# RVC-Project/obs-rvc

Hardware: AMD Instinct MI355X
Metric: audio frames/sec (10 ms hops of new input, 160 ms chunks @16 kHz) (higher is better)
Workload: dtype f32; 1 GPU; BASELINE configs[1]: 1 stream(s)/GPU, ContentVec v2-768 + RMVPE + NSF-HiFiGAN v2-48k, retrieval off, preset full; streams_per_gpu=1, streams_total=1, hip_graph=False

## Files before the change

include/rvc_mi355x_debug.h:

```cpp
#ifndef RVC_MI355X_DEBUG_H
#define RVC_MI355X_DEBUG_H
#include "rvc_mi355x.h"
#ifdef __cplusplus
extern "C" {
#endif

int rvc_debug_option(const char *name, const char *value);
int rvc_debug_stamps(rvc_engine *e, char *buf, size_t cap);
int rvc_debug_last_plan(rvc_engine *e, int *n_ops);
int rvc_debug_profile_dump(rvc_engine *e, char *buf, size_t cap);
double rvc_debug_conv_check(rvc_engine *e, int M, int Cin, int KW, int dil, int N, int streams, int pre_act);
double rvc_debug_conv2d_check(rvc_engine *e, int M, int Cin, int H, int W, int streams, int kind, int residual);
double rvc_debug_ln_fold_check(rvc_engine *e, int M, int K, int N, float offset);
typedef struct rvc_debug_layer_spec {
    int form, streams;
    int cin, cout, kw, stride, pad, dil, groups;
    int t_in, t_out, x_halo, y_halo, r_halo;
    int act; float slope; float scale; int accumulate;
    int pre_act; float pre_slope;
    int no_bias, final_out, glu;
    int res;
    int n, kws[4], dils[4], pads[4];
    int x_grouped, res_grouped, y_ws;
} rvc_debug_layer_spec;
int rvc_debug_layer(rvc_engine *e, const rvc_debug_layer_spec *s, const float *w, const float *bias, float *x, float *y, float *r, long long *geo);
typedef struct rvc_debug_op_spec {
    int op, streams;
    int E, heads, T, window, C, H;
    int x_halo, y_halo;
    int reps, graph;
} rvc_debug_op_spec;
int rvc_debug_op(rvc_engine *e, const rvc_debug_op_spec *s, const float *w0, const float *w1, float *x, float *y, int *status, long long *geo);
typedef struct rvc_debug_stream_state {
    float uppower; unsigned stream_id, chunk; int status;
    float cache_pitchf[1024];
} rvc_debug_stream_state;
typedef struct rvc_debug_front_spec {
    int op, streams, graph;
    int n, frame;
    float bn_scale, bn_shift;
    int C, L;
    int Tm, update, shift, cache_start, read_start, R;
    int T, upp, x_halo, f0_num, f0_den;
    float sr, lin_w, lin_b;
    unsigned seed;
} rvc_debug_front_spec;
int rvc_debug_front(rvc_engine *e, const rvc_debug_front_spec *s, const float *w0, const float *w1, float *const *buf, rvc_debug_stream_state *state, long long *geo);
int rvc_debug_autotune_dump(char *buf, size_t cap);
void rvc_debug_autotune_reset(void);
int rvc_debug_weight_slabs(int device, int *count, size_t *bytes);
const char *rvc_debug_last_kernel(void);
int rvc_debug_formant_table(size_t o, size_t n, float *out, size_t cap, size_t *width);
float rvc_debug_session_sola_ms(rvc_session *s, int enable);

#ifdef __cplusplus
}
#endif
#endif
```

obs_rvc_amd/csrc/engine.hip:

```cpp
#include "engine_int.h"
#include "../../include/rvc_mi355x_debug.h"
#include "crossfade.hip.h"
#include <chrono>

static bool g_planted_queues = false;
__attribute__((constructor)) static void rvc_runtime_defaults()
{
    if (getenv("RVC_NO_RUNTIME_DEFAULTS")) return;
    if (!getenv("GPU_MAX_HW_QUEUES")) { setenv("GPU_MAX_HW_QUEUES", "16", 0); g_planted_queues = true; }
}

namespace rvc {

static void init_kernel_attrs()
{
    static std::mutex mu; static bool done[64] = {};
    int dev = 0; HIPCHK(hipGetDevice(&dev));
    std::lock_guard<std::mutex> lk(mu);
    if (dev >= 0 && dev < 64) { if (done[dev]) return; done[dev] = true; }
    plan_kernel_attrs(); retrieval_kernel_attrs();
}

static void init_constants(rvc_engine *e)
{
// ... 1107 lines not shown
        HIPCHK(hipEventRecord(b, e->stream));
        HIPCHK(hipStreamSynchronize(e->stream));
        float ms; HIPCHK(hipEventElapsedTime(&ms, a, b));
        us = ms * 1e3 / iters;
        (void)hipEventDestroy(a); (void)hipEventDestroy(b);
        free_conv(cw);
        return RVC_OK;
    });
    return us;
}
#endif

double rvc_debug_ln_fold_check(rvc_engine *e, int M, int K, int N, float offset)
{
    double worst = -1.0;
    (void)guarded(e, [&]() {
        if (K % 16 != 0) throw ShapeError("K must be a multiple of 16");
        auto rnd = [](size_t i, unsigned salt) { return (float)((((i + 1) * 2654435761u) ^ (salt * 40503u) ^ (i >> 5)) % 2001) / 1000.0f - 1.0f; };
        std::vector<float> w1((size_t)M * K), b1(M), w2((size_t)K * M), b2(K), g(K), beta(K), hx((size_t)K * N), hz((size_t)M * N);
        for (size_t i = 0; i < w1.size(); i++) w1[i] = 0.5f * rnd(i, 1);
        for (size_t i = 0; i < w2.size(); i++) w2[i] = 0.5f * rnd(i, 2);
        for (int m = 0; m < M; m++) b1[m] = 0.1f * rnd(m, 3);
        for (int k = 0; k < K; k++) { b2[k] = 0.1f * rnd(k, 4); g[k] = 1.0f + 0.3f * rnd(k, 5); beta[k] = 0.2f * rnd(k, 6); }
        for (size_t i = 0; i < hx.size(); i++) hx[i] = 2.0f * rnd(i, 7) + offset;
        for (size_t i = 0; i < hz.size(); i++) hz[i] = rnd(i, 8);
        float *wsum = nullptr;
        ConvW c1 = ModelCV::fold_ln(w1.data(), b1.data(), M, K, g.data(), beta.data(), &wsum);
        ConvW c2 = prep_conv(w2.data(), b2.data(), K, M, 1, 1);
        float *dg = upload_f(g), *dbeta = upload_f(beta);
        Plan pl; pl.B = 1;
        T1 x = make_t1(pl.arena, 1, K, N, 0), y1 = make_t1(pl.arena, 1, M, N, 0), z = make_t1(pl.arena, 1, M, N, 0), y2 = make_t1(pl.arena, 1, K, N, 0);
        float *st = pl.arena.floats((size_t)2 * N + 16);
        for (int k = 0; k < K; k++) HIPCHK(hipMemcpy(x.p + (long long)k * x.ld, &hx[(size_t)k * N], (size_t)N * 4, hipMemcpyHostToDevice));
        for (int m = 0; m < M; m++) HIPCHK(hipMemcpy(z.p + (long long)m * z.ld, &hz[(size_t)m * N], (size_t)N * 4, hipMemcpyHostToDevice));
        { ConvOpts o; o.ln_wsum = wsum; o.ln_stats_out = st; o.ln_rows = K; add_conv1d(pl, c1, x, y1, 1, 0, 1, o); }
        { ConvOpts o; o.res = x.p; o.res_cs = x.ld; o.res_bs = x.bs; o.ln_stats_in = st; o.ln_g = dg; o.ln_b = dbeta; add_conv1d(pl, c2, z, y2, 1, 0, 1, o); }
        HIPCHK(hipDeviceSynchronize());
        for (auto &op : pl.ops.v) op(e->stream);
        HIPCHK(hipStreamSynchronize(e->stream));
        HIPCHK(hipGetLastError());
        std::vector<double> ln((size_t)K * N), mean(N), rstd(N);
        for (int n = 0; n < N; n++) {
            double s = 0; for (int k = 0; k < K; k++) s += hx[(size_t)k * N + n];
            const double mu = s / K; double q = 0;
            for (int k = 0; k < K; k++) { const double d = hx[(size_t)k * N + n] - mu; q += d * d; }
            mean[n] = mu; rstd[n] = 1.0 / std::sqrt(q / K + 1e-5);
            for (int k = 0; k < K; k++) ln[(size_t)k * N + n] = (hx[(size_t)k * N + n] - mu) * rstd[n] * g[k] + beta[k];
        }
        double err = 0.0;
        std::vector<float> row(N), hst((size_t)2 * N);
        {
            double ss = 0; std::vector<double> ref((size_t)M * N);
            for (int m = 0; m < M; m++) for (int n = 0; n < N; n++) {
                double a = b1[m]; for (int k = 0; k < K; k++) a += (double)w1[(size_t)m * K + k] * ln[(size_t)k * N + n];
                ref[(size_t)m * N + n] = a; ss += a * a;
            }
            const double rms1 = std::sqrt(ss / ((double)M * N)) + 1e-12;
            for (int m = 0; m < M; m++) {
                HIPCHK(hipMemcpy(row.data(), y1.p + (long long)m * y1.ld, (size_t)N * 4, hipMemcpyDeviceToHost));
                for (int n = 0; n < N; n++) err = std::max(err, std::fabs((double)row[n] - ref[(size_t)m * N + n]) / rms1);
            }
        }
        {
            double ss = 0; std::vector<double> ref((size_t)K * N);
            for (int k = 0; k < K; k++) for (int n = 0; n < N; n++) {
                double a = b2[k]; for (int m = 0; m < M; m++) a += (double)w2[(size_t)k * M + m] * hz[(size_t)m * N + n];
                a += ln[(size_t)k * N + n];
                ref[(size_t)k * N + n] = a; ss += a * a;
            }
            const double rms2 = std::sqrt(ss / ((double)K * N)) + 1e-12;
            for (int k = 0; k < K; k++) {
                HIPCHK(hipMemcpy(row.data(), y2.p + (long long)k * y2.ld, (size_t)N * 4, hipMemcpyDeviceToHost));
                for (int n = 0; n < N; n++) err = std::max(err, std::fabs((double)row[n] - ref[(size_t)k * N + n]) / rms2);
            }
        }
        HIPCHK(hipMemcpy(hst.data(), st, (size_t)2 * N * 4, hipMemcpyDeviceToHost));
        for (int n = 0; n < N; n++) {
            err = std::max(err, std::fabs((double)hst[2 * n] - mean[n]) / (std::fabs(mean[n]) + 1.0));
            err = std::max(err, std::fabs((double)hst[2 * n + 1] - rstd[n]) / rstd[n]);
        }
        worst = err;
        free_conv(c1); free_conv(c2);
        wfree(wsum); wfree(dg); wfree(dbeta);
        return RVC_OK;
    });
    return worst;
}

#ifdef RVC_TUNING
int rvc_debug_conv_probe(rvc_engine *e, int M, int Cin, int KW, int dil, int N, unsigned long long *out, size_t cap_waves, double *event_us, int *waves_per_wg)
{
    int nw = -1;
    (void)guarded(e, [&]() {
        std::vector<float> w((size_t)M * Cin * KW), bias(M, 0.1f);
        for (size_t i = 0; i < w.size(); i++) w[i] = (float)((i * 2654435761u) % 1000) / 1000.0f - 0.5f;
        ConvW cw = prep_conv(w.data(), bias.data(), M, Cin, KW, 1);
        Plan pl; pl.B = 1;
        const int pad = (KW - 1) * dil / 2;
        T1 x = make_t1(pl.arena, 1, Cin, N, (pad + 3) / 4 * 4), y = make_t1(pl.arena, 1, M, N, 0);
        std::vector<float> hx((size_t)Cin * x.ld, 0.25f);
        HIPCHK(hipMemcpy(x.p - x.halo, hx.data(), hx.size() * 4, hipMemcpyHostToDevice));
        unsigned long long *d_probe; const size_t pbytes = (size_t)1 << 24;
        HIPCHK(hipMalloc(&d_probe, pbytes)); HIPCHK(hipMemset(d_probe, 0, pbytes));
        g_kprobe = d_probe;
        ConvOpts o; if (const char *a = tune_env("RVC_BENCH_ACT")) o.act = atoi(a);
        add_conv1d(pl, cw, x, y, 1, pad, dil, o);
        g_kprobe = nullptr;
        HIPCHK(hipDeviceSynchronize());
        for (int i = 0; i < 5; i++) for (auto &op : pl.ops.v) op(e->stream);
        HIPCHK(hipDeviceSynchronize());
        HIPCHK(hipMemset(d_probe, 0, pbytes));
        HIPCHK(hipDeviceSynchronize());
        pl.profile = true; pl.prof_used = 0;
        for (auto &op : pl.ops.v) op(e->stream);
        HIPCHK(hipDeviceSynchronize());
        float t = 0.f; HIPCHK(hipEventElapsedTime(&t, pl.prof[0].a, pl.prof[0].b));
        if (event_us) *event_us = t * 1e3;
        nw = g_last_wgs * g_last_waves;
        if (waves_per_wg) *waves_per_wg = g_last_waves;
        if ((size_t)nw <= cap_waves && (size_t)nw * 128 <= pbytes) HIPCHK(hipMemcpy(out, d_probe, (size_t)nw * 128, hipMemcpyDeviceToHost));
        else nw = -2;
        (void)hipFree(d_probe);
        free_conv(cw);
        return RVC_OK;
    });
    return nw;
}
#endif

double rvc_debug_conv_check(rvc_engine *e, int M, int Cin, int KW, int dil, int N, int streams, int pre_act)
{
    double worst = -1.0;
    (void)guarded(e, [&]() {
        std::vector<float> w((size_t)M * Cin * KW), bias(M);
        for (size_t i = 0; i < w.size(); i++) w[i] = (float)((i * 2654435761u) % 1000) / 1000.0f - 0.5f;
        for (int m = 0; m < M; m++) bias[m] = 0.01f * (float)(m % 7) - 0.02f;
        ConvW cw = prep_conv(w.data(), bias.data(), M, Cin, KW, 1);
        Plan pl; pl.B = streams;
        const int pad = (KW - 1) * dil / 2, halo = (pad + 3) / 4 * 4;
        T1 x = make_t1(pl.arena, streams, Cin, N, halo), y = make_t1(pl.arena, streams, M, N, 0);
        std::vector<float> hx((size_t)streams * Cin * N);
        for (size_t i = 0; i < hx.size(); i++) hx[i] = (float)(((i * 40503u) ^ (i >> 3)) % 2001) / 1000.0f - 1.0f;
        for (int b = 0; b < streams; b++)
            for (int c = 0; c < Cin; c++)
                HIPCHK(hipMemcpy(x.p + (long long)b * x.bs + (long long)c * x.ld, &hx[((size_t)b * Cin + c) * N], (size_t)N * 4, hipMemcpyHostToDevice));
        ConvOpts o; if (pre_act) { o.pre_act = ACT_LRELU; o.pre_slope = 0.1f; }
        add_conv1d(pl, cw, x, y, 1, pad, dil, o);
        HIPCHK(hipDeviceSynchronize());
        for (auto &op : pl.ops.v) op(e->stream);
        HIPCHK(hipStreamSynchronize(e->stream));
        HIPCHK(hipGetLastError());
        std::vector<float> hy((size_t)streams * M * N);
        for (int b = 0; b < streams; b++)
            HIPCHK(hipMemcpy2D(&hy[(size_t)b * M * N], (size_t)N * 4, y.p + (long long)b * y.bs, (size_t)y.ld * 4, (size_t)N * 4, M, hipMemcpyDeviceToHost));
        const int nthr = (int)std::max(1u, std::min(16u, std::thread::hardware_concurrency()));
        std::vector<double> errs(nthr, 0.0), sss(nthr, 0.0);
        std::vector<std::thread> pool;
        for (int t = 0; t < nthr; t++)
            pool.emplace_back([&, t]() {
                std::vector<double> ref((size_t)N);
                for (long long bm = t; bm < (long long)streams * M; bm += nthr) {
                    const int b = (int)(bm / M), m = (int)(bm % M);
                    for (int n = 0; n < N; n++) {
                        double a = bias[m];
                        for (int c = 0; c < Cin; c++)
                            for (int k = 0; k < KW; k++) {
// ... 445 lines not shown
```

obs_rvc_amd/csrc/engine_int.h:

```cpp
#pragma once
#include "../../include/rvc_mi355x.h"
#include "blob.h"
#include "kernels.hip.h"
#include "formant.hip.h"
#include "igemm_launch.h"
#include <hip/hip_ext.h>

#include <algorithm>
#include <atomic>
#include <cmath>
#include <cstdarg>
#include <cstddef>
#include <functional>
#include <map>
#include <memory>
#include <mutex>
#include <string>
#include <tuple>
#include <vector>
#include <thread>

namespace rvc {

const char *test_opt(const char *name);
// ... 59 lines not shown
    size_t left_ = 0, total_ = 0;
};

struct T1 {
    float *p = nullptr;
    int B = 1, C = 0, T = 0, ld = 0, halo = 0;
    long long bs = 0;
    T1 rows(int c0, int n) const { T1 r = *this; r.p = p + (long long)c0 * ld; r.C = n; return r; }
};
struct T2 {
    float *p = nullptr;
    int B = 1, C = 0, H = 0, W = 0, ld = 0, cs = 0;
    long long bs = 0;
    T2 chans(int c0, int n) const { T2 r = *this; r.p = p + (long long)c0 * cs; r.C = n; return r; }
};

static inline size_t t1_guard(int ld) { return (size_t)ld + 64; }
static inline size_t t2_guard(int ld) { return (size_t)ld * 2 + 64; }
static inline T1 make_t1(Arena &a, int B, int C, int T, int halo)
{
    T1 t;
    t.B = B; t.C = C; t.T = T; t.halo = halo;
    t.ld = (T + 2 * halo + 3) / 4 * 4;
    t.bs = (long long)C * t.ld;
    const size_t guard = t1_guard(t.ld);
    float *base = a.floats((size_t)B * t.bs + 2 * guard);
    t.p = base + guard + halo;
    return t;
}
static inline T2 make_t2(Arena &a, int B, int C, int H, int W)
{
    T2 t;
    t.B = B; t.C = C; t.H = H; t.W = W;
    t.ld = W + 2;
    t.cs = (H + 2) * t.ld;
    t.bs = (long long)C * t.cs;
    const size_t guard = t2_guard(t.ld);
    float *base = a.floats((size_t)B * t.bs + 2 * guard);
    t.p = base + guard + t.ld + 1;
    return t;
}

struct ConvW {
    float *w = nullptr, *bias = nullptr;
    int M = 0, K = 0, Kp = 0, nphase = 1;
    int Cin = 0, Cout = 0, KW = 1, groups = 1;
    int S = 1, ntaps = 1;
    bool transposed = false;
    bool owns = true;
    std::vector<float> host_w;
};

static inline int round16(int k) { return (k + 15) / 16 * 16; }


void *wmalloc(size_t bytes); void wfree(void *p);
void *wmalloc_plan(size_t bytes);
void wslab_info(int dev, int *count, size_t *bytes);
float *upload_f(const std::vector<float> &v, int cls = 0);
float *upload_f(const float *p, size_t n);
float *upload_fragments(const std::vector<float> &panel, int nphase, int M, int Kp, int cls = 0);
static inline long long phase_stride(const ConvW &c) { return (long long)((c.M + 15) / 16 * 16) * c.Kp; }
ConvW prep_conv(const float *w, const float *bias, int Cout, int Cin, int KW, int groups);
ConvW prep_convT1d(const float *w, const float *bias, int Cin, int Cout, int K, int S);
ConvW prep_convT2d(const float *w, const float *bias, int Cin, int Cout);
void free_conv(ConvW &c);
const float *c32s_panel(const float *src_frag, int M, int nchunks, int cin, int KW);
void merge_convs(const std::vector<ConvW *> &cs);

constexpr int LN_FOLD_MAX_STREAMS = 1;

struct ConvOpts {
    int act = ACT_NONE; float slope = 0.f; float scale = 1.f; bool accumulate = false;
    int pre_act = ACT_NONE; float pre_slope = 0.f;
    const float *res = nullptr; int res_cs = 0; long long res_bs = 0; int res_rs = 0;
    int m_off = 0, m_cnt = -1;
    bool no_bias = false;
    bool glu = false;
    bool bf3 = false;
    int y_ws = 0;
    bool final_out = false;
    const float *ln_wsum = nullptr; float *ln_stats_out = nullptr; int ln_rows = 0;
    const float *ln_stats_in = nullptr, *ln_g = nullptr, *ln_b = nullptr;
};

struct ProfEvent { hipEvent_t a, b; double flops; double bytes; int desc = -1; };

struct Plan;
typedef std::function<void(hipStream_t)> Op;

struct TapRec { std::string name; int rank; T1 t1; T2 t2; };

struct OpList {
    std::vector<Op> v;
    std::vector<int> sid;
    std::vector<int> kind;
    std::vector<int> order_eager, order_graph;
    int cur = 0;
    void push_back(Op o) { v.push_back(std::move(o)); sid.push_back(cur); kind.push_back(0); }
    void fork(int s) { v.push_back(Op()); sid.push_back(s); kind.push_back(1); }
    void join(int s) { v.push_back(Op()); sid.push_back(s); kind.push_back(2); }
};

struct Plan {
    Arena arena;
    OpList ops;
    std::vector<TapRec> taps;
    int B = 1; size_t L = 0, frame16k = 0; uint32_t skip_head = 0, R = 0;
    int T = 0, Tm = 0, C = 0; size_t N = 0;
    bool with_index = false, with_taps = false;
    bool bucket = false;
    std::map<std::vector<int>, const int *> koff_tabs;
    bool rm_fuse = false;
    bool bf3 = false;
    bool autotune = false;
    double tune_ms = 0; int tuned_layers = 0, tune_changed = 0, tune_hits = 0;
    bool plain_plan = false;
    int mode = 0;
    uint32_t R2 = 0; bool fstage = false;
    int dec_frames() const { return fstage ? (int)R2 : (int)R; }
    float *d_in = nullptr;
    T1 cv_out, audio;
    float *d_f0 = nullptr;
    float *d_feat = nullptr;
    int *d_knn_idx = nullptr; float *d_knn_dist = nullptr;
    unsigned *knn_ticket = nullptr; size_t knn_ticket_bytes = 0;
    std::vector<Op> knn_fallback;
    size_t op_phone = 0, op_ret_begin = 0, op_ret_end = 0;
    unsigned opt_gen = 0;
    bool profile = false;
    std::vector<ProfEvent> prof;
    std::vector<std::string> descs;
    size_t prof_used = 0;
    double igemm_flops = 0;
    int n_igemm = 0;
    std::vector<float *> owned_dev;
    unsigned long long *d_stamps = nullptr; std::vector<std::string> stamp_names;
    int slot = 0; hipEvent_t ev_done = nullptr; bool ev_done_valid = false;
    const float *cur_in = nullptr; float *cur_out = nullptr; long long cur_out_bs = 0;
    bool in_direct_ok = true, out_direct_ok = false;
    bool final_out_honoured = false;
    hipGraphExec_t graph_exec = nullptr;
    ProfEvent *prof_slot(double flops, double bytes, int desc)
    {
        if (!profile) return nullptr;
        if (prof_used == prof.size()) { ProfEvent e; HIPCHK(hipEventCreate(&e.a)); HIPCHK(hipEventCreate(&e.b)); prof.push_back(e); }
        ProfEvent *pe = &prof[prof_used++];
        pe->flops = flops; pe->bytes = bytes; pe->desc = desc;
        return pe;
    }
    ~Plan()
    {
        for (float *p : owned_dev) wfree(p);
        if (graph_exec) (void)hipGraphExecDestroy(graph_exec);
        if (ev_done) (void)hipEventDestroy(ev_done);
        for (auto &e : prof) { (void)hipEventDestroy(e.a); (void)hipEventDestroy(e.b); }
    }
};


extern unsigned long long *g_kprobe;
extern int g_last_waves, g_last_wgs, g_ncu;
extern thread_local char g_last_kernel[32];
void queue_igemm(Plan &pl, IgemmP p, int B, const std::vector<int> &koff, const std::vector<PhaseD> &phases, bool final_out = false);
template <class Launch> void queue_gemm_launch(Plan &pl, const char *desc, double flops, int wgs, int waves, bool final_out, const IgemmP &p, Launch launch);
void fill_epilogue(IgemmP &p, const ConvW &cw, const ConvOpts &o);
void add_conv1d(Plan &pl, const ConvW &cw, const T1 &x, const T1 &y, int stride, int pad, int dil, ConvOpts o = ConvOpts());
void add_conv1d_multi(Plan &pl, const std::vector<const ConvW *> &cws, const T1 &x, bool x_grouped, const T1 &y,
                      const std::vector<int> &pads, const std::vector<int> &dils, ConvOpts o = ConvOpts(), bool res_grouped = true);
void add_conv1d_two(Plan &pl, const ConvW &c0, const ConvW &c1, const float *pair_bias, const T1 &x, const T1 &y0, const T1 &y1);
void add_convT1d(Plan &pl, const ConvW &cw, const T1 &x, const T1 &y, int pad, ConvOpts o = ConvOpts());
void add_conv2d(Plan &pl, const ConvW &cw, const T2 &x, const T2 &y, ConvOpts o = ConvOpts());
void add_convT2d(Plan &pl, const ConvW &cw, const T2 &x, const T2 &y, ConvOpts o = ConvOpts());
void add_layernorm(Plan &pl, const T1 &x, const float *g, const float *b);
void add_attention(Plan &pl, const T1 &qkv, const T1 &out, int heads);
void add_relpos_attention(Plan &pl, const T1 &qkv, const T1 &out, int heads, const float *rel_k, const float *rel_v, int window);
void add_gru(Plan &pl, const T1 &gi, const T1 &out, int H, const float *whh, const float *whhT, const float *bhh, int *status, int status_stride);
void add_stamp(Plan &pl, const char *name);
void add_tap(Plan &pl, const char *name, const T1 &t);
void add_tap2(Plan &pl, const char *name, const T2 &t);
void plan_kernel_attrs();
void retrieval_kernel_attrs();

struct DevVec { float *p = nullptr; };
static inline float *dv(const Blob &b, const std::string &name) { const BlobTensor &t = b.t(name); return upload_f(t.data, t.nelem); }

struct ModelCV {
    int conv_dim, embed, heads, ffn, run_layers, pos_k, pos_groups, out_dim;
    int conv_k[7], conv_s[7];
    ConvW conv[7], proj, pos, final_proj;
    float *gn_g, *gn_b, *ln0_g, *ln0_b, *encln_g, *encln_b;
    float *conv0_raw = nullptr;
    struct Layer { ConvW qkv, o, ff1, ff2, qkv_f, ff1_f; float *qkv_wsum = nullptr, *ff1_wsum = nullptr; float *ln1_g, *ln1_b, *ln2_g, *ln2_b; };
    bool has_folded = false;
    ConvW proj_f; float *proj_wsum = nullptr;
    static ConvW fold_ln(const float *w, const float *bias, int M, int K, const float *g, const float *beta, float **wsum_dev)
    {
        std::vector<float> wf((size_t)M * K), bf(M), ws(M);
        for (int m = 0; m < M; m++) {
            double sb = bias ? bias[m] : 0.0, sw = 0.0;
            for (int k = 0; k < K; k++) {
                const float v = w[(size_t)m * K + k] * g[k];
                wf[(size_t)m * K + k] = v;
                sb += (double)w[(size_t)m * K + k] * beta[k];
                sw += v;
            }
            bf[m] = (float)sb; ws[m] = (float)sw;
        }
        *wsum_dev = upload_f(ws);
        return prep_conv(wf.data(), bf.data(), M, K, 1, 1);
    }
    std::vector<Layer> layers;
    std::vector<float *> owned;
    size_t weight_bytes = 0;
    explicit ModelCV(const Blob &b)
    {
        conv_dim = b.icfg("conv_dim"); embed = b.icfg("embed"); heads = b.icfg("heads"); ffn = b.icfg("ffn");
        run_layers = b.icfg("run_layers"); pos_k = b.icfg("pos_k"); pos_groups = b.icfg("pos_groups"); out_dim = b.icfg("out_dim");
        int cin = 1;
        for (int i = 0; i < 7; i++) {
            conv_k[i] = b.icfg(fmt("conv_k%d", i)); conv_s[i] = b.icfg(fmt("conv_s%d", i));
            conv[i] = prep_conv(b.w(fmt("cv.conv%d.w", i)), nullptr, conv_dim, cin, conv_k[i], 1);
            cin = conv_dim;
        }
        auto own = [&](const std::string &n) { float *p = dv(b, n); owned.push_back(p); return p; };
        conv0_raw = own("cv.conv0.w");
        gn_g = own("cv.gn.g"); gn_b = own("cv.gn.b"); ln0_g = own("cv.ln0.g"); ln0_b = own("cv.ln0.b");
        proj = prep_conv(b.w("cv.proj.w"), b.w("cv.proj.b"), embed, conv_dim, 1, 1);
        pos = prep_conv(b.w("cv.pos.w"), b.w("cv.pos.b"), embed, embed, pos_k, pos_groups);
        encln_g = own("cv.enc_ln.g"); encln_b = own("cv.enc_ln.b");
        const int E = embed;
        for (int l = 0; l < run_layers; l++) {
            Layer L;
            std::vector<float> w((size_t)3 * E * E), bb((size_t)3 * E);
            const char *nm[3] = {"q", "k", "v"};
            for (int j = 0; j < 3; j++) {
                memcpy(&w[(size_t)j * E * E], b.w(fmt("cv.l%d.", l) + nm[j] + ".w"), (size_t)E * E * 4);
                memcpy(&bb[(size_t)j * E], b.w(fmt("cv.l%d.", l) + nm[j] + ".b"), (size_t)E * 4);
            }
            L.qkv = prep_conv(w.data(), bb.data(), 3 * E, E, 1, 1);
            L.o = prep_conv(b.w(fmt("cv.l%d.o.w", l)), b.w(fmt("cv.l%d.o.b", l)), E, E, 1, 1);
            L.ff1 = prep_conv(b.w(fmt("cv.l%d.ff1.w", l)), b.w(fmt("cv.l%d.ff1.b", l)), ffn, E, 1, 1);
            L.ff2 = prep_conv(b.w(fmt("cv.l%d.ff2.w", l)), b.w(fmt("cv.l%d.ff2.b", l)), E, ffn, 1, 1);
            L.ln1_g = own(fmt("cv.l%d.ln1.g", l)); L.ln1_b = own(fmt("cv.l%d.ln1.b", l));
            L.ln2_g = own(fmt("cv.l%d.ln2.g", l)); L.ln2_b = own(fmt("cv.l%d.ln2.b", l));
            if (E >= 256 && E % 64 == 0 && ffn % 64 == 0 && !test_opt("RVC_NO_LN_FUSE")) {
                has_folded = true;
                L.ff1_f = fold_ln(b.w(fmt("cv.l%d.ff1.w", l)), b.w(fmt("cv.l%d.ff1.b", l)), ffn, E, b.w(fmt("cv.l%d.ln1.g", l)), b.w(fmt("cv.l%d.ln1.b", l)), &L.ff1_wsum);
                if (l > 0) L.qkv_f = fold_ln(w.data(), bb.data(), 3 * E, E, b.w(fmt("cv.l%d.ln2.g", l - 1)), b.w(fmt("cv.l%d.ln2.b", l - 1)), &L.qkv_wsum);
                else L.qkv_f = fold_ln(w.data(), bb.data(), 3 * E, E, b.w("cv.enc_ln.g"), b.w("cv.enc_ln.b"), &L.qkv_wsum);
            }
            layers.push_back(L);
        }
        if (out_dim != E) final_proj = prep_conv(b.w("cv.final_proj.w"), b.w("cv.final_proj.b"), out_dim, E, 1, 1);
        if (has_folded && conv_dim % 64 == 0) proj_f = fold_ln(b.w("cv.proj.w"), b.w("cv.proj.b"), embed, conv_dim, b.w("cv.ln0.g"), b.w("cv.ln0.b"), &proj_wsum);
        weight_bytes = b.bytes();
    }
// ... 73 lines not shown
            r.f_w1 = upload_f(all); r.f_w2 = r.f_w1 + o2; r.f_sc = r.has_sc ? r.f_w1 + o3 : nullptr; r.f_lines = (int)(all.size() / 32);
        }
        return r;
    }
    explicit ModelRM(const Blob &b)
    {
        en_out = b.icfg("en_out"); levels = b.icfg("levels"); n_blocks = b.icfg("n_blocks"); inter_layers = b.icfg("inter_layers");
        n_mels = b.icfg("n_mels"); gru_hidden = b.icfg("gru_hidden"); n_out = b.icfg("n_out");
        bn_scale = b.w("rm.bn0")[0]; bn_shift = b.w("rm.bn0")[1];
        int ci = 1, co = en_out;
        for (int lv = 0; lv < levels; lv++) {
            std::vector<ResBlockW> v;
            for (int j = 0; j < n_blocks; j++) v.push_back(block(b, fmt("rm.enc%d.b%d.", lv, j), j == 0 ? ci : co, co));
            enc.push_back(v);
            ci = co; co *= 2;
        }
        for (int lv = 0; lv < inter_layers; lv++) {
            std::vector<ResBlockW> v;
            for (int j = 0; j < n_blocks; j++) v.push_back(block(b, fmt("rm.int%d.b%d.", lv, j), j == 0 ? (lv == 0 ? ci : co) : co, co));
            inter.push_back(v);
        }
        ci = co;
        for (int lv = 0; lv < levels; lv++) {
            co = ci / 2;
            up.push_back(prep_convT2d(b.w(fmt("rm.dec%d.up.w", lv)), b.w(fmt("rm.dec%d.up.b", lv)), ci, co));
            std::vector<ResBlockW> v;
            for (int j = 0; j < n_blocks; j++) v.push_back(block(b, fmt("rm.dec%d.b%d.", lv, j), j == 0 ? 2 * co : co, co));
            dec.push_back(v);
            ci = co;
        }
        cnn = prep_conv(b.w("rm.cnn.w"), b.w("rm.cnn.b"), 3, en_out, 9, 1);
        const int H = gru_hidden, I = 3 * n_mels;
        std::vector<float> wih((size_t)6 * H * I), bih((size_t)6 * H), bh((size_t)6 * H);
        const char *sfx[2] = {"f", "b"};
        const float *whh_dir[2];
        for (int d = 0; d < 2; d++) {
            memcpy(&wih[(size_t)d * 3 * H * I], b.w(std::string("rm.gru.w_ih_") + sfx[d]), (size_t)3 * H * I * 4);
            memcpy(&bih[(size_t)d * 3 * H], b.w(std::string("rm.gru.b_ih_") + sfx[d]), (size_t)3 * H * 4);
            memcpy(&bh[(size_t)d * 3 * H], b.w(std::string("rm.gru.b_hh_") + sfx[d]), (size_t)3 * H * 4);
            whh_dir[d] = b.w(std::string("rm.gru.w_hh_") + sfx[d]);
        }
        gru_ih = prep_conv(wih.data(), bih.data(), 6 * H, I, 1, 1);
        {
            std::vector<float> wt, wr;
            gru_prep_whh(whh_dir, H, wt, wr);
            whhT = upload_f(wt); bhh = upload_f(bh); whh = upload_f(wr);
        }
        fc = prep_conv(b.w("rm.fc.w"), b.w("rm.fc.b"), n_out, 2 * H, 1, 1);
        weight_bytes = b.bytes();
    }
    ~ModelRM()
    {
        auto fb = [](std::vector<std::vector<ResBlockW>> &vv) { for (auto &v : vv) for (auto &r : v) { free_conv(r.c1); free_conv(r.c2); free_conv(r.sc); if (r.pair_bias) wfree(r.pair_bias); if (r.f_w1) wfree(r.f_w1); } };
        fb(enc); fb(inter); fb(dec);
        for (auto &u : up) free_conv(u);
        free_conv(cnn); free_conv(gru_ih); free_conv(fc);
        if (whhT) wfree(whhT);
        if (bhh) wfree(bhh);
        if (whh) wfree(whh);
    }
};

template <typename T> static inline void glu_pack_rows(const T *w, const float *bias, int H, size_t K, std::vector<float> &wp, std::vector<float> &bp)
{
    if (H % 8 != 0) throw std::runtime_error("GLU-gated layer: channel count must be a multiple of 8");
    wp.resize((size_t)2 * H * K); bp.resize((size_t)2 * H);
    for (int r = 0; r < 2 * H; r++) {
        const int f = r >> 4, kq = (r & 15) >> 2, rr = r & 3;
        const int src = f * 8 + kq * 2 + (rr & 1) + (rr >= 2 ? H : 0);
        for (size_t q = 0; q < K; q++) wp[(size_t)r * K + q] = (float)w[(size_t)src * K + q];
        bp[r] = bias[src];
    }
}

struct ModelSY {
    int phone_dim, hidden, inter, filter, heads, enc_layers, enc_k, window, flow_n, wn_layers, wn_k, gin, up_init, n_ups, n_rb, n_rbd, sr;
    int up_rate[8], up_kernel[8], rb_k[8], rb_d[8];
    ConvW phone, proj;
    float *pitch_emb = nullptr;
    struct Layer {
        ConvW qkv, o, ff1, ff2, qkv_f; float *qkv_wsum = nullptr; float *rel_k, *rel_v, *ln1_g, *ln1_b, *ln2_g, *ln2_b;
    };
    ConvW proj_f; float *proj_wsum = nullptr; bool has_folded = false;
    std::vector<Layer> layers;
    struct Flow {
        ConvW pre, post; std::vector<ConvW> in, rs; bool flipped = false;
        std::vector<float> h_pre_w, h_pre_b, h_post_w, h_post_b;
        std::vector<std::vector<float>> h_in_w, h_in_b, h_rs_w, h_rs_b;
        ConvW pre1, postc, posth; std::vector<ConvW> inc; float *pair_bias = nullptr;
    };
    bool composed = false;
    std::vector<Flow> flows;
    ConvW dec_pre, dec_post;
    std::vector<ConvW> ups, ncs;
    std::vector<std::vector<std::vector<std::pair<ConvW, ConvW>>>> rbs;
    float src_w, src_b;
    std::vector<float *> owned;
    size_t weight_bytes = 0;
    explicit ModelSY(const Blob &b)
    {
        phone_dim = b.icfg("phone_dim"); hidden = b.icfg("hidden"); inter = b.icfg("inter"); filter = b.icfg("filter"); heads = b.icfg("heads");
        enc_layers = b.icfg("enc_layers"); enc_k = b.icfg("enc_k"); window = b.icfg("window"); flow_n = b.icfg("flow_n");
        wn_layers = b.icfg("wn_layers"); wn_k = b.icfg("wn_k"); gin = b.icfg("gin"); up_init = b.icfg("up_init"); n_ups = b.icfg("n_ups");
        n_rb = b.icfg("n_rb"); n_rbd = b.icfg("n_rbd"); sr = b.icfg("sr");
        for (int i = 0; i < n_ups; i++) { up_rate[i] = b.icfg(fmt("up_rate%d", i)); up_kernel[i] = b.icfg(fmt("up_kernel%d", i)); }
        for (int j = 0; j < n_rb; j++) rb_k[j] = b.icfg(fmt("rb_k%d", j));
        for (int m = 0; m < n_rbd; m++) rb_d[m] = b.icfg(fmt("rb_d%d", m));
        auto own = [&](const std::string &n) { float *p = dv(b, n); owned.push_back(p); return p; };
        const int H = hidden, G = gin;
        const float *g = b.w("sy.g");
        phone = prep_conv(b.w("sy.enc.phone.w"), b.w("sy.enc.phone.b"), H, phone_dim, 1, 1);
        pitch_emb = own("sy.enc.pitch_emb");
        for (int l = 0; l < enc_layers; l++) {
            Layer L;
            std::vector<float> w((size_t)3 * H * H), bb((size_t)3 * H);
            const char *nm[3] = {"q", "k", "v"};
            for (int j = 0; j < 3; j++) {
                memcpy(&w[(size_t)j * H * H], b.w(fmt("sy.enc.l%d.", l) + nm[j] + ".w"), (size_t)H * H * 4);
                memcpy(&bb[(size_t)j * H], b.w(fmt("sy.enc.l%d.", l) + nm[j] + ".b"), (size_t)H * 4);
            }
            L.qkv = prep_conv(w.data(), bb.data(), 3 * H, H, 1, 1);
            L.o = prep_conv(b.w(fmt("sy.enc.l%d.o.w", l)), b.w(fmt("sy.enc.l%d.o.b", l)), H, H, 1, 1);
            L.ff1 = prep_conv(b.w(fmt("sy.enc.l%d.ff1.w", l)), b.w(fmt("sy.enc.l%d.ff1.b", l)), filter, H, enc_k, 1);
            L.ff2 = prep_conv(b.w(fmt("sy.enc.l%d.ff2.w", l)), b.w(fmt("sy.enc.l%d.ff2.b", l)), H, filter, enc_k, 1);
            L.rel_k = own(fmt("sy.enc.l%d.rel_k", l)); L.rel_v = own(fmt("sy.enc.l%d.rel_v", l));
            L.ln1_g = own(fmt("sy.enc.l%d.ln1.g", l)); L.ln1_b = own(fmt("sy.enc.l%d.ln1.b", l));
            L.ln2_g = own(fmt("sy.enc.l%d.ln2.g", l)); L.ln2_b = own(fmt("sy.enc.l%d.ln2.b", l));
            if (H >= 128 && H % 16 == 0 && !test_opt("RVC_NO_LN_FUSE")) {
                has_folded = true;
                if (l > 0) L.qkv_f = ModelCV::fold_ln(w.data(), bb.data(), 3 * H, H, b.w(fmt("sy.enc.l%d.ln2.g", l - 1)), b.w(fmt("sy.enc.l%d.ln2.b", l - 1)), &L.qkv_wsum);
            }
            layers.push_back(L);
        }
        proj = prep_conv(b.w("sy.enc.proj.w"), b.w("sy.enc.proj.b"), 2 * inter, H, 1, 1);
        if (has_folded)
            proj_f = ModelCV::fold_ln(b.w("sy.enc.proj.w"), b.w("sy.enc.proj.b"), 2 * inter, H, b.w(fmt("sy.enc.l%d.ln2.g", enc_layers - 1)), b.w(fmt("sy.enc.l%d.ln2.b", enc_layers - 1)), &proj_wsum);
        const int half = inter / 2;
        for (int i = 0; i < flow_n; i++) {
            Flow F;
            F.flipped = ((flow_n - i) & 1) != 0;
            {
                std::vector<float> w((size_t)2 * H * half, 0.f), bb((size_t)2 * H, 0.f);
                const float *pw = b.w(fmt("sy.flow%d.pre.w", i)), *pb = b.w(fmt("sy.flow%d.pre.b", i));
                for (int r = 0; r < H; r++) {
                    bb[r] = pb[r];
                    for (int q = 0; q < half; q++) w[(size_t)r * half + q] = pw[(size_t)r * half + (F.flipped ? half - 1 - q : q)];
                }
                F.pre = prep_conv(w.data(), bb.data(), 2 * H, half, 1, 1);
                F.h_pre_w.assign(w.begin(), w.begin() + (size_t)H * half); F.h_pre_b.assign(bb.begin(), bb.begin() + H);
            }
            const float *cw = b.w(fmt("sy.flow%d.cond.w", i)), *cb = b.w(fmt("sy.flow%d.cond.b", i));
            for (int j = 0; j < wn_layers; j++) {
                std::vector<float> bias(2 * H);
                const float *ib = b.w(fmt("sy.flow%d.in%d.b", i, j));
                for (int r = 0; r < 2 * H; r++) {
                    float a = cb[j * 2 * H + r];
                    for (int q = 0; q < G; q++) a += cw[(size_t)(j * 2 * H + r) * G + q] * g[q];
                    bias[r] = ib[r] + a;
                }
                {
                    const float *iw = b.w(fmt("sy.flow%d.in%d.w", i, j));
                    const size_t Kin = (size_t)H * wn_k;
                    std::vector<float> w, pb;
                    glu_pack_rows(iw, bias.data(), H, Kin, w, pb);
                    F.in.push_back(prep_conv(w.data(), pb.data(), 2 * H, H, wn_k, 1));
                    F.h_in_w.emplace_back(iw, iw + (size_t)2 * H * Kin); F.h_in_b.push_back(bias);
                }
                int rs_c = j < wn_layers - 1 ? 2 * H : H;
                F.rs.push_back(prep_conv(b.w(fmt("sy.flow%d.rs%d.w", i, j)), b.w(fmt("sy.flow%d.rs%d.b", i, j)), rs_c, H, 1, 1));
                { const float *rw = b.w(fmt("sy.flow%d.rs%d.w", i, j)), *rb = b.w(fmt("sy.flow%d.rs%d.b", i, j)); F.h_rs_w.emplace_back(rw, rw + (size_t)rs_c * H); F.h_rs_b.emplace_back(rb, rb + rs_c); }
            }
            {
                const float *pw = b.w(fmt("sy.flow%d.post.w", i)), *pb = b.w(fmt("sy.flow%d.post.b", i));
                std::vector<float> w((size_t)half * H), bb(half);
                for (int r = 0; r < half; r++) {
                    const int src = F.flipped ? half - 1 - r : r;
                    memcpy(&w[(size_t)r * H], pw + (size_t)src * H, (size_t)H * sizeof(float));
                    bb[r] = pb[src];
                }
                F.post = prep_conv(w.data(), bb.data(), half, H, 1, 1);
                F.h_post_w = w; F.h_post_b = bb;
            }
            flows.push_back(F);
        }
        if (hidden % 16 == 0 && inter == hidden && !test_opt("RVC_NO_WN_COMPOSE")) compose_flows();
        {
            std::vector<float> bias(up_init);
            const float *cw = b.w("sy.dec.cond.w"), *cb = b.w("sy.dec.cond.b"), *pb = b.w("sy.dec.pre.b");
            for (int c = 0; c < up_init; c++) { float a = cb[c]; for (int q = 0; q < G; q++) a += cw[(size_t)c * G + q] * g[q]; bias[c] = pb[c] + a; }
            dec_pre = prep_conv(b.w("sy.dec.pre.w"), bias.data(), up_init, inter, 7, 1);
        }
        int c = up_init;
        for (int i = 0; i < n_ups; i++) {
            int co = c / 2;
            ups.push_back(prep_convT1d(b.w(fmt("sy.dec.up%d.w", i)), b.w(fmt("sy.dec.up%d.b", i)), c, co, up_kernel[i], up_rate[i]));
            int sf = 1; for (int q = i + 1; q < n_ups; q++) sf *= up_rate[q];
            int nk = i + 1 < n_ups ? 2 * sf : 1;
            ncs.push_back(prep_conv(b.w(fmt("sy.dec.nc%d.w", i)), b.w(fmt("sy.dec.nc%d.b", i)), co, 1, nk, 1));
            std::vector<std::vector<std::pair<ConvW, ConvW>>> stage;
            for (int j = 0; j < n_rb; j++) {
                std::vector<std::pair<ConvW, ConvW>> chain;
                for (int m = 0; m < n_rbd; m++) {
                    ConvW c1 = prep_conv(b.w(fmt("sy.dec.rb%d_%d.c1_%d.w", i, j, m)), b.w(fmt("sy.dec.rb%d_%d.c1_%d.b", i, j, m)), co, co, rb_k[j], 1);
                    ConvW c2 = prep_conv(b.w(fmt("sy.dec.rb%d_%d.c2_%d.w", i, j, m)), b.w(fmt("sy.dec.rb%d_%d.c2_%d.b", i, j, m)), co, co, rb_k[j], 1);
                    chain.push_back({c1, c2});
                }
                stage.push_back(chain);
            }
            rbs.push_back(stage);
            for (int m = 0; m < n_rbd && n_rb > 1; m++) {
                std::vector<ConvW *> a, bb;
                for (int j = 0; j < n_rb; j++) { a.push_back(&rbs.back()[j][m].first); bb.push_back(&rbs.back()[j][m].second); }
                merge_convs(a); merge_convs(bb);
            }
            c = co;
        }
        dec_post = prep_conv(b.w("sy.dec.post.w"), nullptr, 1, c, 7, 1);
        src_w = b.w("sy.src")[0]; src_b = b.w("sy.src")[1];
        weight_bytes = b.bytes();
// ... 35 lines not shown
                        }
                }
                std::vector<float> wp, pb;
                glu_pack_rows(w.data(), F.h_in_b[j].data(), H, (size_t)Cin * K5, wp, pb);
                WJ[fi][j] = std::move(wp); BJ[fi][j] = std::move(pb);
            }
        };
        auto one_flow = [&](int fi) {
            Flow &F = flows[fi];
            WP1[fi].assign((size_t)H * I, 0.f); BP1[fi] = F.h_pre_b;
            for (int r = 0; r < H; r++) for (int q = 0; q < half; q++) WP1[fi][(size_t)r * I + x0_row0(F) + q] = F.h_pre_w[(size_t)r * half + q];
            const int KA = nl * H, Kin = KA + I;
            std::vector<double> pc((size_t)half * KA, 0.0), pcb(half, 0.0);
            for (int r = 0; r < half; r++) {
                double bacc = F.h_post_b[r];
                for (int j = 0; j < nl; j++) {
                    const int row0 = j < nl - 1 ? H : 0;
                    const float *S = F.h_rs_w[j].data() + (size_t)row0 * H, *sb = F.h_rs_b[j].data() + row0;
                    for (int h = 0; h < H; h++) {
                        const double v = F.h_post_w[(size_t)r * H + h];
                        for (int c = 0; c < H; c++) pc[(size_t)r * KA + (size_t)j * H + c] += v * S[(size_t)h * H + c];
                        bacc += v * sb[h];
                    }
                }
                pcb[r] = bacc;
            }
            const bool has_next = fi > 0;
            const int r1 = x1_row0(F);
            std::vector<double> wz((size_t)I * Kin, 0.0), bz(I, 0.0);
            for (int c = 0; c < I; c++) wz[(size_t)c * Kin + KA + c] = 1.0;
            for (int r = 0; r < half; r++) {
                for (int q = 0; q < KA; q++) wz[(size_t)(r1 + r) * Kin + q] = -pc[(size_t)r * KA + q];
                bz[r1 + r] = -pcb[r];
            }
            WM[fi].resize(wz.size()); BM[fi].resize(I);
            for (size_t q = 0; q < wz.size(); q++) WM[fi][q] = (float)wz[q];
            for (int r = 0; r < I; r++) BM[fi][r] = (float)bz[r];
            if (has_next) {
                const Flow &N = flows[fi - 1];
                std::vector<double> wh((size_t)H * Kin, 0.0);
                WH[fi].resize(wh.size()); BH[fi].resize(H);
                for (int r = 0; r < H; r++) {
                    double bacc = N.h_pre_b[r];
                    for (int q = 0; q < half; q++) {
                        const double v = N.h_pre_w[(size_t)r * half + q];
                        const int zc = x0_row0(N) + q;
                        wh[(size_t)r * Kin + KA + zc] += v;
                        if (zc >= r1 && zc < r1 + half) {
                            const int pr = zc - r1;
                            for (int c = 0; c < KA; c++) wh[(size_t)r * Kin + c] -= v * pc[(size_t)pr * KA + c];
                            bacc -= v * pcb[pr];
                        }
                    }
                    BH[fi][r] = (float)bacc;
                }
                for (size_t q = 0; q < wh.size(); q++) WH[fi][q] = (float)wh[q];
            }
        };
        for (int i = 0; i < nfl; i++) { WJ[i].resize(nl); BJ[i].resize(nl); }
        std::vector<std::thread> th;
        for (int i = 0; i < nfl; i++) {
            th.emplace_back([&, i]() { one_flow(i); });
            for (int j = 0; j < nl; j++) th.emplace_back([&, i, j]() { in_layer(i, j); });
        }
        for (auto &t : th) t.join();
        for (int i = 0; i < nfl; i++) {
            Flow &F = flows[i];
            F.pre1 = prep_conv(WP1[i].data(), BP1[i].data(), H, I, 1, 1);
            for (int j = 0; j < nl; j++) F.inc.push_back(prep_conv(WJ[i][j].data(), BJ[i][j].data(), 2 * H, 16 + H * (j + 1), K5, 1));
            F.postc = prep_conv(WM[i].data(), BM[i].data(), I, nl * H + I, 1, 1);
            if (i > 0) {
                F.posth = prep_conv(WH[i].data(), BH[i].data(), H, nl * H + I, 1, 1);
                std::vector<float> pb(BH[i]); pb.insert(pb.end(), BM[i].begin(), BM[i].end());
                F.pair_bias = upload_f(pb); owned.push_back(F.pair_bias);
            }
        }
        composed = true;
    }
    ~ModelSY()
    {
        free_conv(phone); free_conv(proj); free_conv(dec_pre); free_conv(dec_post);
        for (auto &L : layers) { free_conv(L.qkv); free_conv(L.o); free_conv(L.ff1); free_conv(L.ff2); free_conv(L.qkv_f); if (L.qkv_wsum) wfree(L.qkv_wsum); }
        free_conv(proj_f); if (proj_wsum) wfree(proj_wsum);
        for (auto &F : flows) { free_conv(F.pre); free_conv(F.post); for (auto &c : F.in) free_conv(c); for (auto &c : F.rs) free_conv(c); if (composed) { free_conv(F.pre1); free_conv(F.postc); free_conv(F.posth); for (auto &c : F.inc) free_conv(c); } }
        for (auto &c : ups) free_conv(c);
        for (auto &c : ncs) free_conv(c);
        for (auto &s : rbs) for (auto &ch : s) for (auto &pr : ch) { free_conv(pr.first); free_conv(pr.second); }
        for (float *p : owned) wfree(p);
    }
    int upp() const { int u = 1; for (int i = 0; i < n_ups; i++) u *= up_rate[i]; return u; }
};

}

namespace rvc { struct StreamSet; }
using namespace rvc;

struct rvc_engine {
    std::string data_path, err;
    int device = 0;
    hipStream_t stream = nullptr, aux[3] = {nullptr, nullptr, nullptr};
    struct rvc::StreamSet *sset = nullptr;
    int cv_cus = 256;
    bool partition_ok = false, partitioned = false;
    hipEvent_t ev_fork[3] = {nullptr, nullptr, nullptr}, ev_join[3] = {nullptr, nullptr, nullptr};
    std::unique_ptr<ModelCV> cv;
    std::unique_ptr<ModelRM> rm;
    std::unique_ptr<ModelSY> sy;
    float *d_window = nullptr, *d_twiddle = nullptr, *d_basis = nullptr; int *d_band = nullptr;
    float *d_index = nullptr, *d_indexT = nullptr, *d_indexF = nullptr, *d_ynorm = nullptr, *d_nhn = nullptr; size_t index_n = 0, index_dim = 0; bool index_owned = true;
    float index_rate = 0.f;
    float index_prep_ms = 0.f;
    double bcast_ms[3] = {0, 0, 0}; int bcast_ranks = 0;
    int n_streams = 1;
    StreamState *d_state = nullptr;
    StreamState *d_state_bucket = nullptr; int *d_bucket_idx = nullptr;
    CallParams *d_cp = nullptr, *h_cp = nullptr;
    unsigned cp_slot = 0; hipEvent_t ev_cp = nullptr;
    uint32_t seed = 0, stream_id0 = 0;
    std::vector<std::unique_ptr<Plan>> plans;
    Plan *last_plan = nullptr;
    int gemm_precision = 0;
    int plan_cap = 8;
    int autotune = 1;
    double last_build_ms = 0;
    int last_tuned = 0, last_changed = 0, last_hits = 0; double last_tune_ms = 0;
    long long knn_recoveries = 0;
    long long plan_builds = 0;
    int taps_on = 0;
    bool profile_on = false, use_graph = false;
    bool pipeline = false, pipe_now = false; int pipe_slot = 0; hipEvent_t ev_in = nullptr; const void *pipe_input = nullptr; size_t pipe_input_bytes = 0;
    std::vector<float> pushed_up; uint32_t pushed_seed = 0; bool pushed_valid = false;
    float *h_up = nullptr; unsigned up_slot = 0;
    hipEvent_t ev_up[8] = {nullptr, nullptr, nullptr, nullptr, nullptr, nullptr, nullptr, nullptr}; bool ev_up_used[8] = {false, false, false, false, false, false, false, false};
    hipEvent_t ev0 = nullptr, ev1 = nullptr;
    float last_ms = 0.f;
    size_t last_knn_rows = 0;
    std::vector<double> formant; double formant_default = 0.0;
    std::map<std::pair<int, int>, rvc::FormantTable> ftabs;
    std::vector<rvc::FormantDesc> pushed_fd;
    rvc::FormantDesc *h_fd = nullptr;
    int *h_status = nullptr;
    bool status_queued = false;
};


namespace rvc {
static inline void set_device(rvc_engine *e) { HIPCHK(hipSetDevice(e->device)); }
template <typename Fn> static rvc_status guarded(rvc_engine *e, Fn fn)
{
    if (!e) return RVC_BACKEND;
    try {
        set_device(e);
        return fn();
    } catch (const ShapeError &x) { e->err = x.what(); return RVC_SHAPE; }
    catch (const PanicError &x) { e->err = x.what(); return RVC_PANIC; }
    catch (const std::exception &x) { e->err = x.what(); return RVC_BACKEND; }
}
T1 build_contentvec(rvc_engine *e, Plan &pl, int B, size_t L);
T1 build_rmvpe(rvc_engine *e, Plan &pl, int B, size_t L, size_t frame16k, bool update_cache);
void build_pitch_post(rvc_engine *e, Plan &pl, int B, const T1 &sal, bool update_cache, size_t frame16k, size_t hubert_length, float **pitchf_out, int **pitch_out);
T1 build_nsf_source(rvc_engine *e, Plan &pl, int B, float *d_pitchf);
void add_conv0_front(Plan &pl, const ConvW &cw, const float *w_raw, const float *gn_g, const float *gn_b, int kt, int st, const T1 &x, const T1 &y);
void add_mel_frontend(rvc_engine *e, Plan &pl, int B, const float *audio, long long audio_bs, int n, int frame, int Tm, float *mel, const T2 &img, float bn_scale, float bn_shift);
void add_pitch_post(Plan &pl, int B, const T1 &sal, int Tm, StreamState *st, const CallParams *cp, float *f0, bool update, long long shift, long long cache_start,
                    long long read_start, int R, float *pitchf, int *pitch);
// ... 9 lines not shown
```

obs_rvc_amd/csrc/igemm.hip.h:

```cpp
#pragma once
#include <hip/hip_runtime.h>
#include <stdint.h>

namespace rvc {

typedef float f32x4 __attribute__((ext_vector_type(4)));

enum Act { ACT_NONE = 0, ACT_RELU = 1, ACT_LRELU = 2, ACT_GELU = 3, ACT_TANH = 4, ACT_SIGMOID = 5 };

#ifdef RVC_FAST_GELU
__device__ __forceinline__ float erf_dev(float x)
{
    x = fminf(fmaxf(x, -4.f), 4.f);
    const float x2 = x * x;
    float p = -2.72614225801306e-10f;
    p = fmaf(p, x2, 2.77068142495902e-08f); p = fmaf(p, x2, -2.10102402082508e-06f); p = fmaf(p, x2, -5.69250639462346e-05f);
    p = fmaf(p, x2, -7.34990630326855e-04f); p = fmaf(p, x2, -2.95459980854025e-03f); p = fmaf(p, x2, -1.60960333262415e-02f);
    float q = -1.45660718464996e-05f;
    q = fmaf(q, x2, -2.13374055278905e-04f); q = fmaf(q, x2, -1.68282697438203e-03f); q = fmaf(q, x2, -7.37332916720468e-03f); q = fmaf(q, x2, -1.42647390514189e-02f);
    return x * p * __builtin_amdgcn_rcpf(q);
}
#else
__device__ __forceinline__ float erf_dev(float x) { return erff(x); }
#endif
__device__ __forceinline__ float gelu_dev(float v) { return 0.5f * v * (1.0f + erf_dev(v * 0.70710678118654752440f)); }

__device__ __forceinline__ float apply_act(float v, int act, float slope)
{
    switch (act) {
    case ACT_RELU: return v > 0.f ? v : 0.f;
    case ACT_LRELU: return v > 0.f ? v : v * slope;
    case ACT_GELU: return gelu_dev(v);
    case ACT_TANH: return tanhf(v);
    case ACT_SIGMOID: return 1.0f / (1.0f + expf(-v));
    default: return v;
    }
}

struct PhaseD {
    long long w_off;
    int x_off;
    int y_c0;
    int y_h0;
    int y_pos;
    int bias_off;
    int koff_off;
    int nchunks;
    int act_p1;
    int pad_;
    long long y_off;
    int t_tab;
    int t_cin;
    int t_rs;
    int t_dmin;
};

struct IgemmP {
    const float *x, *w, *bias, *res;
    float *y, *part;
    const int *koff;
    const PhaseD *ph;
    PhaseD ph0;
    int M, N, K;
    int NW;
    int x_hs, x_ws;
    int y_hm, y_ws;
    int OW;
    long long x_bs, y_bs, res_bs;
    int y_cs, res_cs;
    int y_rs, res_rs;
    int nphase, ksplit, chunks_per_split;
    int act; float slope; float scale; int accumulate;
    int pre_act; float pre_slope;
    int ntn, ntm;
    int koff_bias;
    int glu;
    int res_nogroup;
    unsigned long long *probe;
    int m_fast;
    int nbatch;
    int fold_n;
    int bf3;
    int lin_cs4;
    const float *ln_wsum;
    float *ln_stats_out;
    const float *ln_stats_in, *ln_g, *ln_bt;
    float ln_eps, ln_inv_rows;
    const int *items, *ttab;
    int x_ld, x_lo, x_lim, pad2_;
};

__device__ __forceinline__ void epilogue_store(const IgemmP &p, const PhaseD &ph, int b, int m, int n, float acc)
{
    if (m >= p.M || n >= p.N) return;
    if (p.fold_n) { b = n / p.fold_n; n -= b * p.fold_n; }
    int nh = 0, nw = n;
    if (p.y_hm) { nh = n / p.NW; nw = n - nh * p.NW; }
    const int ow = nw * p.y_ws + ph.y_pos, oh = nh * p.y_hm + ph.y_h0;
    if (ow < 0 || ow >= p.OW) return;
    const int ch = m + ph.y_c0;
    float v = acc;
    if (p.bias) v += p.bias[ph.bias_off + m];
    v = apply_act(v, p.act, p.slope);
    if (p.res) v += p.res[(long long)b * p.res_bs + (long long)(p.res_nogroup ? m : ch) * p.res_cs + (long long)oh * p.res_rs + ow];
    v *= p.scale;
    float *yp = p.y + (long long)b * p.y_bs + (long long)ch * p.y_cs + (long long)oh * p.y_rs + ow;
    if (p.accumulate) v += *yp;
    *yp = v;
}

__device__ __forceinline__ void glu_store(const IgemmP &p, const PhaseD &ph, int b, int m1, int n, float a1, float a2)
{
    if (m1 >= p.M || n >= p.N) return;
    if (p.fold_n) { b = n / p.fold_n; n -= b * p.fold_n; }
    const float ta = a1 + p.bias[ph.bias_off + m1], sa = a2 + p.bias[ph.bias_off + m1 + 2];
    const int ch = (m1 >> 4) * 8 + ((m1 & 15) >> 2) * 2 + (m1 & 1) + ph.y_c0;
    p.y[(long long)b * p.y_bs + (long long)ch * p.y_cs + n] = tanhf(ta) * (1.0f / (1.0f + expf(-sa)));
}

struct EpiPre { float bias, res, yold; };
__device__ __forceinline__ bool epi_locate(const IgemmP &p, const PhaseD &ph, int m, int n, int &ch, int &oh, int &ow)
{
    if (m >= p.M || n >= p.N) return false;
    int nh = 0, nw = n;
    if (p.y_hm) { nh = n / p.NW; nw = n - nh * p.NW; }
    ow = nw * p.y_ws + ph.y_pos; oh = nh * p.y_hm + ph.y_h0;
    if (ow < 0 || ow >= p.OW) return false;
    ch = m + ph.y_c0;
    return true;
}
__device__ __forceinline__ EpiPre epi_prefetch(const IgemmP &p, const PhaseD &ph, int b, int m, int n)
{
    EpiPre e = {0.f, 0.f, 0.f};
    int ch, oh, ow;
    if (!epi_locate(p, ph, m, n, ch, oh, ow)) return e;
    if (p.bias) e.bias = p.bias[ph.bias_off + m];
    if (p.res) e.res = p.res[(long long)b * p.res_bs + (long long)(p.res_nogroup ? m : ch) * p.res_cs + (long long)oh * p.res_rs + ow];
    if (p.accumulate) e.yold = p.y[(long long)b * p.y_bs + (long long)ch * p.y_cs + (long long)oh * p.y_rs + ow];
    return e;
}
__device__ __forceinline__ void epi_finish(const IgemmP &p, const PhaseD &ph, int b, int m, int n, float acc, const EpiPre &e)
{
    int ch, oh, ow;
    if (!epi_locate(p, ph, m, n, ch, oh, ow)) return;
    float v = apply_act(acc + e.bias, p.act, p.slope);
    v += e.res;
    v *= p.scale;
    v += e.yold;
    p.y[(long long)b * p.y_bs + (long long)ch * p.y_cs + (long long)oh * p.y_rs + ow] = v;
}

__device__ __forceinline__ void lds_only_barrier()
{
    __builtin_amdgcn_s_waitcnt(0xC07F);
    __builtin_amdgcn_s_barrier();
}

#ifdef RVC_KPROBE
#define RVC_KP(i) do { if (p.probe && (threadIdx.x & 63) == 0) p.probe[((size_t)((blockIdx.z * gridDim.y + blockIdx.y) * gridDim.x + blockIdx.x) * (blockDim.x >> 6) + (threadIdx.x >> 6)) * 16 + (i)] = wall_clock64(); } while (0)
#else
#define RVC_KP(i)
#endif
template <int MF, int NF, int D, int KS, bool PRE>
__global__ __launch_bounds__((KS > 1 ? KS : 4) * 64) void igemm_kernel(IgemmP p)
{
    constexpr int WAVES = KS > 1 ? KS : 4;
    RVC_KP(0);
    constexpr int NACC = (MF * NF == 1) ? 2 : 1;
    constexpr int TE = MF * NF * 256;
    constexpr int PE = (KS > 1) ? ((TE + WAVES * 64 - 1) / (WAVES * 64)) : 1;
    constexpr bool PF = (KS > 1) || (MF * NF <= 4);
    extern __shared__ __attribute__((aligned(16))) int s_koff[];
    const int lane = threadIdx.x & 63, wave = threadIdx.x >> 6;
    const int tile = KS > 1 ? (int)blockIdx.x : (int)blockIdx.x * 4 + wave;
    int z = blockIdx.y;
    const int ks = z % p.ksplit; z /= p.ksplit;
    const int phase = z % p.nphase;
    const int b = z / p.nphase;
    const PhaseD ph = p.nphase == 1 ? p.ph0 : p.ph[phase];
    const int nchunks = ph.nchunks;
    const int g0 = ks * p.chunks_per_split;
    int g1 = g0 + p.chunks_per_split;
    g1 = g1 < nchunks ? g1 : nchunks;
    const int gn = g1 - g0;
    {
        const int4 *src = reinterpret_cast<const int4 *>(p.koff + ph.koff_off + g0 * 16);
        int4 *dst = reinterpret_cast<int4 *>(s_koff);
        for (int i = threadIdx.x; i < gn * 4; i += WAVES * 64) dst[i] = src[i];
    }
    RVC_KP(8);
    int tn, tm;
    if (p.m_fast) { tm = tile % p.m_fast; tn = tile / p.m_fast; }
    else { tn = tile % p.ntn; tm = tile / p.ntn; }
    const bool live = tm < p.ntm && tn < p.ntn;
    const int li = lane & 15, kq = lane >> 4;

    EpiPre pre_w[(KS > 1 || !PF) ? 1 : MF][(KS > 1 || !PF) ? 1 : NF][4];
    EpiPre pre_r[PE];
    if (PF && live && p.ksplit == 1) {
        if (KS > 1) {
// ... 158 lines not shown
            }
            if (p.ksplit == 1) epi_finish(p, ph, b, m, n, v, pre_r[q]);
            else if (m < p.M && n < p.N)
                p.part[(((long long)(b * p.nphase + phase) * p.ksplit + ks) * p.M + m) * (long long)p.N + n] = v;
        }
        RVC_KP(6);
        return;
    }
    if (p.glu) {
#pragma unroll
        for (int mf = 0; mf < MF; mf++)
#pragma unroll
            for (int nf = 0; nf < NF; nf++)
#pragma unroll
                for (int r = 0; r < 2; r++)
                    glu_store(p, ph, b, tm * 16 * MF + mf * 16 + kq * 4 + r, tn * 16 * NF + nf * 16 + li, acc[0][mf][nf][r], acc[0][mf][nf][r + 2]);
        return;
    }
    if (p.ksplit == 1) {
#pragma unroll
        for (int mf = 0; mf < MF; mf++)
#pragma unroll
            for (int nf = 0; nf < NF; nf++)
#pragma unroll
                for (int r = 0; r < 4; r++) {
                    const int m = tm * 16 * MF + mf * 16 + kq * 4 + r, n = tn * 16 * NF + nf * 16 + li;
                    if (PF) epi_finish(p, ph, b, m, n, acc[0][mf][nf][r], pre_w[PF ? mf : 0][PF ? nf : 0][r]);
                    else epilogue_store(p, ph, b, m, n, acc[0][mf][nf][r]);
                }
        RVC_KP(6);
    } else {
        float *pp = p.part + ((long long)(b * p.nphase + phase) * p.ksplit + ks) * (long long)p.M * p.N;
#pragma unroll
        for (int mf = 0; mf < MF; mf++)
#pragma unroll
            for (int nf = 0; nf < NF; nf++)
#pragma unroll
                for (int r = 0; r < 4; r++) {
                    int m = tm * 16 * MF + mf * 16 + kq * 4 + r, n = tn * 16 * NF + nf * 16 + li;
                    if (m < p.M && n < p.N) pp[(long long)m * p.N + n] = acc[0][mf][nf][r];
                }
    }
}

__device__ __forceinline__ int xcd_tile_id(int x, int gx, int row_start)
{
    const int off = row_start & 7, c = (x + off) & 7;
    int base = 0;
#pragma unroll
    for (int cc = 0; cc < 8; cc++) {
        const int f = (cc - off) & 7;
        const int cnt = f < gx ? (gx - f + 7) >> 3 : 0;
        base += cc < c ? cnt : 0;
    }
    return base + ((x - ((c - off) & 7)) >> 3);
}

template <int ACT> __device__ __forceinline__ float act_t(float v, float slope)
{
    if (ACT == ACT_RELU) return v > 0.f ? v : 0.f;
    if (ACT == ACT_LRELU) return v > 0.f ? v : v * slope;
    if (ACT == ACT_GELU) return gelu_dev(v);
    if (ACT == ACT_TANH) return tanhf(v);
    if (ACT == ACT_SIGMOID) return 1.0f / (1.0f + expf(-v));
    return v;
}
struct Epi2 { float bias, res, yold; int yo; };
__device__ __forceinline__ Epi2 epi2_prefetch(const IgemmP &p, const PhaseD &ph, const float *resb, const float *yb, int m, int n)
{
    Epi2 e = {0.f, 0.f, 0.f, -1};
    if (m >= p.M || n >= p.N) return e;
    const int n_launch = n;
    int bb = 0;
    if (p.fold_n) { bb = n / p.fold_n; n -= bb * p.fold_n; }
    int nh = 0, nw = n;
    if (p.y_hm) { nh = n / p.NW; nw = n - nh * p.NW; }
    const int ow = nw * p.y_ws + ph.y_pos, oh = nh * p.y_hm + ph.y_h0;
    if (ow < 0 || ow >= p.OW) return e;
    const int ch = m + ph.y_c0;
    e.yo = bb * (int)p.y_bs + ch * p.y_cs + oh * p.y_rs + ow;
    if (p.bias) e.bias = p.bias[ph.bias_off + m];
    if (resb) {
        const int rrow = p.res_nogroup ? m : ch;
        e.res = resb[bb * (int)p.res_bs + rrow * p.res_cs + oh * p.res_rs + ow];
        if (p.ln_stats_in)
            e.res = (e.res - p.ln_stats_in[2 * n_launch]) * p.ln_stats_in[2 * n_launch + 1] * p.ln_g[rrow] + p.ln_bt[rrow];
    }
    if (p.accumulate) e.yold = yb[e.yo];
    return e;
}
template <int ACT> __device__ __forceinline__ float epi2_value(float acc, float bias, float res, float yold, float slope, float scale)
{
    float v = act_t<ACT>(acc + bias, slope);
    v += res;
    v *= scale;
    v += yold;
    return v;
}
template <int ACT> __device__ __forceinline__ void epi2_finish(const IgemmP &p, float *yb, float acc, const Epi2 &e)
{
    if (e.yo < 0) return;
    yb[e.yo] = epi2_value<ACT>(acc, e.bias, e.res, e.yold, p.slope, p.scale);
}
struct ColOut { int yo, ro; };
__device__ __forceinline__ ColOut col_locate(const IgemmP &p, const PhaseD &ph, int n)
{
    ColOut c = {-1, 0};
    if (n >= p.N) return c;
    int bb = 0;
    if (p.fold_n) { bb = n / p.fold_n; n -= bb * p.fold_n; }
    int nh = 0, nw = n;
    if (p.y_hm) { nh = n / p.NW; nw = n - nh * p.NW; }
    const int ow = nw * p.y_ws + ph.y_pos, oh = nh * p.y_hm + ph.y_h0;
    if (ow < 0 || ow >= p.OW) return c;
    c.yo = bb * (int)p.y_bs + oh * p.y_rs + ow;
    c.ro = bb * (int)p.res_bs + oh * p.res_rs + ow;
    return c;
}
__device__ __forceinline__ Epi2 epi2_from_col(const IgemmP &p, const PhaseD &ph, const float *resb, const float *yb, const ColOut &c, int m)
{
    Epi2 e = {0.f, 0.f, 0.f, -1};
    if (m >= p.M || c.yo < 0) return e;
    const int ch = m + ph.y_c0;
    e.yo = c.yo + ch * p.y_cs;
    if (p.bias) e.bias = p.bias[ph.bias_off + m];
    if (resb) e.res = resb[c.ro + (p.res_nogroup ? m : ch) * p.res_cs];
    if (p.accumulate) e.yold = yb[e.yo];
    return e;
}
__device__ __forceinline__ Epi2 epi2_plain(float bias, int yo) { Epi2 e = {bias, 0.f, 0.f, yo}; return e; }
__device__ __forceinline__ Epi2 epi2_none() { Epi2 e = {0.f, 0.f, 0.f, -1}; return e; }
__device__ __forceinline__ Epi2 epi2_aux(const IgemmP &p, const PhaseD &ph, const float *resb, const float *yb, const ColOut &c, int m, float bias)
{
    Epi2 e = {bias, 0.f, 0.f, -1};
    if (m >= p.M || c.yo < 0) return e;
    const int ch = m + ph.y_c0;
    e.yo = c.yo + ch * p.y_cs;
    if (resb) e.res = resb[c.ro + (p.res_nogroup ? m : ch) * p.res_cs];
    if (p.accumulate) e.yold = yb[e.yo];
    return e;
}
__device__ __forceinline__ void glu_from_col(const IgemmP &p, const PhaseD &ph, float *yb, const ColOut &c, int m1, float a1, float a2)
{
    if (m1 >= p.M || c.yo < 0) return;
    const float ta = a1 + p.bias[ph.bias_off + m1], sa = a2 + p.bias[ph.bias_off + m1 + 2];
    const int ch = (m1 >> 4) * 8 + ((m1 & 15) >> 2) * 2 + (m1 & 1) + ph.y_c0;
    yb[c.yo + ch * p.y_cs] = tanhf(ta) * (1.0f / (1.0f + expf(-sa)));
}

__device__ __forceinline__ void glu_from_col_b(const IgemmP &p, const PhaseD &ph, float *yb, const ColOut &c, int m1, float a1, float a2, float b1, float b2)
{
    if (m1 >= p.M || c.yo < 0) return;
    const float ta = a1 + b1, sa = a2 + b2;
    const int ch = (m1 >> 4) * 8 + ((m1 & 15) >> 2) * 2 + (m1 & 1) + ph.y_c0;
    yb[c.yo + ch * p.y_cs] = tanhf(ta) * (1.0f / (1.0f + expf(-sa)));
}

#define RVC_ACT_DISPATCH(STMT) RVC_ACT_DISPATCH_SEL(p.act, STMT)
#define RVC_ACT_DISPATCH_SEL(SEL, STMT)                                          \
    switch (SEL) {                                                             \
    case ACT_RELU: { constexpr int A_ = ACT_RELU; STMT } break;                  \
    case ACT_LRELU: { constexpr int A_ = ACT_LRELU; STMT } break;                \
    case ACT_GELU: { constexpr int A_ = ACT_GELU; STMT } break;                  \
    case ACT_TANH: { constexpr int A_ = ACT_TANH; STMT } break;                  \
    case ACT_SIGMOID: { constexpr int A_ = ACT_SIGMOID; STMT } break;            \
    default: { constexpr int A_ = ACT_NONE; STMT } break;                        \
    }
// ... 197 lines not shown
#pragma unroll
                for (int s = 0; s < D; s++) RVC_FUSED_STAGE(s, c + s + D)
            }
        } else {
            for (; c + 2 * D <= nc; c += D) {
#pragma unroll
                for (int s = 0; s < D; s++) {
                    RVC_COMPUTE_STAGE(s)
                    __builtin_amdgcn_sched_barrier(0);
                    RVC_LOAD_STAGE(s, c + s + D)
                    __builtin_amdgcn_sched_barrier(0);
                }
            }
        }
        const int rem = nc - c - D;
#pragma unroll
        for (int s = 0; s < D; s++) {
            RVC_COMPUTE_STAGE(s)
            if (s < rem) RVC_LOAD_STAGE(s, c + s + D)
        }
#pragma unroll
        for (int s = 0; s < D; s++) {
            if (s < rem) RVC_COMPUTE_STAGE(s)
        }
    } else {
        if (live) {
#pragma unroll
            for (int s = 0; s < D; s++)
                if (s < nc) { RVC_LOAD_A(s, s) if (LIN) RVC_LOAD_B(s, s) }
        }
        RVC_EPI_PREFETCH
        RVC_KP(11);
        RVC_PUBLISH_TABLE
        RVC_KP(1);
        if (!live) { if (KS > 1) {  } return; }
        if (!LIN) {
            ko_nx = nc > 0 ? kol[0] : make_int4(0, 0, 0, 0);
#pragma unroll
            for (int s = 0; s < D; s++)
                if (s < nc) RVC_LOAD_B(s, s)
        }
        RVC_KP(2);
#pragma unroll
        for (int s = 0; s < D; s++) {
            if (s < nc) RVC_COMPUTE_STAGE(s)
        }
    }
#undef RVC_FUSED_STAGE
#undef RVC_EPI_PREFETCH
#undef RVC_PUBLISH_TABLE
#undef RVC_COMPUTE_STAGE
#undef RVC_LOAD_STAGE
#undef RVC_LOAD_A
#undef RVC_LOAD_B
    if (NACC == 2) {
#pragma unroll
        for (int mf = 0; mf < MF; mf++)
#pragma unroll
            for (int nf = 0; nf < NF; nf++) acc[0][mf][nf] += acc[NACC - 1][mf][nf];
    }
    RVC_KP(3);

    if (KS > 1) {
        float *red = reinterpret_cast<float *>(s_koff + (LIN ? 0 : nchunks * 16));
#pragma unroll
        for (int mf = 0; mf < MF; mf++)
#pragma unroll
            for (int nf = 0; nf < NF; nf++)
#pragma unroll
                for (int r = 0; r < 4; r++) red[wave * TE + ((mf * NF + nf) * 4 + r) * 64 + lane] = acc[0][mf][nf][r];
        float *lst = red + KS * TE;
        if (LNB) {
#pragma unroll
            for (int nf = 0; nf < NF; nf++) {
                float s_ = ln_s[LNB ? nf : 0], q_ = ln_ss[LNB ? nf : 0];
                s_ += __shfl_xor(s_, 16, 64); q_ += __shfl_xor(q_, 16, 64);
                s_ += __shfl_xor(s_, 32, 64); q_ += __shfl_xor(q_, 32, 64);
                if (kq == 0) { lst[(wave * NF * 16 + nf * 16 + li) * 2] = s_; lst[(wave * NF * 16 + nf * 16 + li) * 2 + 1] = q_; }
            }
        }
        RVC_KP(4);
        __syncthreads();
        RVC_KP(5);
        if (p.glu) {
#pragma unroll
            for (int q = 0; q < PE; q++) {
                const int e = threadIdx.x + q * WAVES * 64;
                if (e >= TE) break;
                const int l = e & 63, r = (e >> 6) & 3, f = e >> 8, mf = f / NF, nf = f - mf * NF;
                if (r >= 2) continue;
                float v = 0.f, v2 = 0.f;
#pragma unroll
                for (int w = 0; w < KS; w++) { v += red[w * TE + e]; v2 += red[w * TE + e + 128]; }
                glu_store(p, ph, b, tm * 16 * MF + mf * 16 + (l >> 4) * 4 + r, tn * 16 * NF + nf * 16 + (l & 15), v, v2);
            }
            return;
        }
        float ln_mean[LNB ? NF : 1], ln_rstd[LNB ? NF : 1];
        if (LNB) {
#pragma unroll
            for (int nf = 0; nf < NF; nf++) {
                const int cl = nf * 16 + li;
                float s_ = 0.f, q_ = 0.f;
#pragma unroll
                for (int w = 0; w < KS; w++) { s_ += lst[(w * NF * 16 + cl) * 2]; q_ += lst[(w * NF * 16 + cl) * 2 + 1]; }
                const float msh = s_ * p.ln_inv_rows;
                const float var = fmaxf(q_ * p.ln_inv_rows - msh * msh, 0.f);
                const float mean = ln_c[LNB ? nf : 0] + msh;
                const float rstd = 1.0f / sqrtf(var + p.ln_eps);
                ln_mean[LNB ? nf : 0] = mean; ln_rstd[LNB ? nf : 0] = rstd;
                const int n_ = tn * 16 * NF + cl;
                if (p.ln_stats_out && tm == 0 && threadIdx.x < 16 && n_ < p.N) { p.ln_stats_out[2 * n_] = mean; p.ln_stats_out[2 * n_ + 1] = rstd; }
            }
        }
        float vsum[PE];
#pragma unroll
        for (int q = 0; q < PE; q++) {
            const int e = threadIdx.x + q * WAVES * 64;
            float v = 0.f;
            if (e < TE) {
#pragma unroll
                for (int w = 0; w < KS; w++) v += red[w * TE + e];
            }
            if (LNB && e < TE) {
                const int nf = (e >> 8) % NF;
                v = ln_rstd[LNB ? nf : 0] * (v - ln_mean[LNB ? nf : 0] * pre_ws[LNB ? q : 0]);
            }
            vsum[q] = v;
        }
        RVC_ACT_DISPATCH_SEL(act_sel, 
            _Pragma("unroll") for (int q = 0; q < PE; q++) epi2_finish<A_>(p, yb, vsum[q], pre_r[q]);
        )
        RVC_KP(6);
        return;
    }
    if (p.glu) {
        float gb[MF][4];
#pragma unroll
        for (int mf = 0; mf < MF; mf++)
#pragma unroll
            for (int r = 0; r < 4; r++) {
                const int m = tm * 16 * MF + mf * 16 + kq * 4 + r;
                gb[mf][r] = m < p.M ? p.bias[ph.bias_off + m] : 0.f;
            }
#pragma unroll
        for (int nf = 0; nf < NF; nf++) {
            const ColOut col = col_locate(p, ph, tn * 16 * NF + nf * 16 + li);
#pragma unroll
            for (int mf = 0; mf < MF; mf++)
#pragma unroll
                for (int r = 0; r < 2; r++)
                    glu_from_col_b(p, ph, yb, col, tm * 16 * MF + mf * 16 + kq * 4 + r, acc[0][mf][nf][r], acc[0][mf][nf][r + 2], gb[mf][r], gb[mf][r + 2]);
        }
        return;
    }
    if (PF) {
        RVC_ACT_DISPATCH_SEL(act_sel, 
            _Pragma("unroll") for (int mf = 0; mf < MF; mf++)
                _Pragma("unroll") for (int nf = 0; nf < NF; nf++)
                    _Pragma("unroll") for (int r = 0; r < 4; r++)
                        epi2_finish<A_>(p, yb, acc[0][mf][nf][r], pre_w[PF ? mf : 0][PF ? nf : 0][r]);
        )
    } else {
        ColOut cols[NF];
#pragma unroll
        for (int nf = 0; nf < NF; nf++) cols[nf] = col_locate(p, ph, tn * 16 * NF + nf * 16 + li);
        const bool has_aux = resb != nullptr || p.accumulate;
        if (!p.accumulate && (tm + 1) * 16 * MF <= p.M) {
            const float slope = p.slope, scale = p.scale;
            const long long cs = p.y_cs, rcs = p.res_cs;
            RVC_ACT_DISPATCH_SEL(act_sel, 
                _Pragma("unroll") for (int mf = 0; mf < MF; mf++) {
                    const int m0 = tm * 16 * MF + mf * 16 + kq * 4;
                    float bias_r[4];
                    _Pragma("unroll") for (int r = 0; r < 4; r++) bias_r[r] = p.bias ? p.bias[ph.bias_off + m0 + r] : 0.f;
                    float rr[NF][4];
                    _Pragma("unroll") for (int nf = 0; nf < NF; nf++)
                        _Pragma("unroll") for (int r = 0; r < 4; r++) rr[nf][r] = 0.f;
                    if (resb) {
                        _Pragma("unroll") for (int nf = 0; nf < NF; nf++)
                            if (cols[nf].yo >= 0) {
                                const float *rp = resb + cols[nf].ro + (long long)(p.res_nogroup ? m0 : m0 + ph.y_c0) * rcs;
                                _Pragma("unroll") for (int r = 0; r < 4; r++) rr[nf][r] = rp[r * rcs];
                            }
                    }
                    _Pragma("unroll") for (int nf = 0; nf < NF; nf++)
                        if (cols[nf].yo >= 0) {
                            float *yc = yb + cols[nf].yo + (long long)(m0 + ph.y_c0) * cs;
                            _Pragma("unroll") for (int r = 0; r < 4; r++)
                                yc[r * cs] = epi2_value<A_>(acc[0][mf][nf][r], bias_r[r], rr[nf][r], 0.f, slope, scale);
                        }
                }
            )
            RVC_KP(6);
            return;
        }
        RVC_ACT_DISPATCH_SEL(act_sel, 
            _Pragma("unroll") for (int mf = 0; mf < MF; mf++) {
                float bias_r[4];
                _Pragma("unroll") for (int r = 0; r < 4; r++) {
                    const int m = tm * 16 * MF + mf * 16 + kq * 4 + r;
                    bias_r[r] = (p.bias && m < p.M) ? p.bias[ph.bias_off + m] : 0.f;
                }
                _Pragma("unroll") for (int nf = 0; nf < NF; nf++) {
                    if (!has_aux) {
                        _Pragma("unroll") for (int r = 0; r < 4; r++) {
                            const int m = tm * 16 * MF + mf * 16 + kq * 4 + r;
                            const Epi2 e1 = epi2_plain(bias_r[r], (m < p.M && cols[nf].yo >= 0) ? cols[nf].yo + (m + ph.y_c0) * p.y_cs : -1);
                            epi2_finish<A_>(p, yb, acc[0][mf][nf][r], e1);
                        }
                    } else {
// ... 708 lines not shown
```

obs_rvc_amd/csrc/kernels.hip.h:

```cpp
#pragma once
#include "igemm.hip.h"
#include "state.hip.h"

namespace rvc {

static __global__ __launch_bounds__(256) void splitk_epilogue_kernel(IgemmP p)
{
    const int total = p.M * p.N;
    const int i = blockIdx.x * blockDim.x + threadIdx.x;
    if (i >= total) return;
    int z = blockIdx.y;
    const int phase = z % p.nphase, b = z / p.nphase;
    const PhaseD ph = p.ph[phase];
    const float *pp = p.part + (long long)(b * p.nphase + phase) * p.ksplit * total + i;
    float acc = 0.f;
    for (int ks = 0; ks < p.ksplit; ks++) acc += pp[(long long)ks * total];
    const int m = i / p.N, n = i - m * p.N;
    epilogue_store(p, ph, b, m, n, acc);
}

__device__ __forceinline__ float wave_sum(float v)
{
#pragma unroll
    for (int o = 32; o > 0; o >>= 1) v += __shfl_xor(v, o, 64);
// ... 93 lines not shown
        }
        const float a0r = vr[0] + vr[2], a0i = vi[0] + vi[2], a1r = vr[0] - vr[2], a1i = vi[0] - vi[2];
        const float a2r = vr[1] + vr[3], a2i = vi[1] + vi[3];
        const float a3r = vi[1] - vi[3], a3i = -(vr[1] - vr[3]);
        const int j0 = (tid / Ns) * Ns * 4 + k;
        float *orr = bufr[cur ^ 1], *oi = bufi[cur ^ 1];
        orr[j0] = a0r + a2r;          oi[j0] = a0i + a2i;
        orr[j0 + Ns] = a1r + a3r;     oi[j0 + Ns] = a1i + a3i;
        orr[j0 + 2 * Ns] = a0r - a2r; oi[j0 + 2 * Ns] = a0i - a2i;
        orr[j0 + 3 * Ns] = a1r - a3r; oi[j0 + 3 * Ns] = a1i - a3i;
        cur ^= 1;
        __syncthreads();
    }
    for (int k = tid; k < 513; k += 256) { const float xr = bufr[cur][k], xi = bufi[cur][k]; mag[k] = sqrtf(xr * xr + xi * xi); }
    __syncthreads();
#pragma unroll
    for (int it = 0; it < 8; it++) {
        const int m = wave * 32 + it * 4 + sub;
        const int lo = blo[it], hi = bhi[it];
        const float *br = p.basis + m * 513;
        float s = 0.f;
#pragma unroll
        for (int j = 0; j < 4; j++) { const int k = lo + l16 + 16 * j; if (k < hi) s += bpre[it][j] * mag[k]; }
        for (int k = lo + l16 + 64; k < hi; k += 16) s += br[k] * mag[k];
        s += __shfl_xor(s, 8, 64); s += __shfl_xor(s, 4, 64); s += __shfl_xor(s, 2, 64); s += __shfl_xor(s, 1, 64);
        if (l16 == 0) {
            const float lm = logf(fmaxf(s, 1e-5f));
            p.mel[((long long)b * 128 + m) * p.Tm + t] = lm;
            p.img[(long long)b * p.img_bs + (long long)t * p.img_ld + m] = lm * p.bn_scale + p.bn_shift;
        }
    }
}

template <int NV>
__global__ __launch_bounds__(256) void layernorm_ct_kernel(const float *x, float *y, const float *g, const float *bta,
                                                           int C, int T, int x_cs, long long x_bs, int y_cs, long long y_bs)
{
    __shared__ float red[4][4];
    const int tx = threadIdx.x & 3, ty = threadIdx.x >> 2;
    const int lane = threadIdx.x & 63, wave = threadIdx.x >> 6;
    const int t = blockIdx.x * 4 + tx, b = blockIdx.y;
    const bool ok = t < T;
    const float *xp = x + (long long)b * x_bs + (ok ? t : 0);
    float v[NV];
    float s = 0.f;
#pragma unroll
    for (int i = 0; i < NV; i++) {
        const int c = ty + i * 64;
        v[i] = (ok && c < C) ? xp[(long long)c * x_cs] : 0.f;
        s += v[i];
    }
    float gv[NV], bv[NV];
#pragma unroll
    for (int i = 0; i < NV; i++) {
        const int c = ty + i * 64;
        gv[i] = c < C ? g[c] : 0.f; bv[i] = c < C ? bta[c] : 0.f;
    }
#pragma unroll
    for (int o = 4; o < 64; o <<= 1) s += __shfl_xor(s, o, 64);
    if (lane < 4) red[wave][lane] = s;
    __syncthreads();
    const float mean = (red[0][tx] + red[1][tx] + red[2][tx] + red[3][tx]) / (float)C;
    __syncthreads();
    float q = 0.f;
#pragma unroll
    for (int i = 0; i < NV; i++) {
        const int c = ty + i * 64;
        const float d = (c < C) ? v[i] - mean : 0.f;
        q += d * d;
    }
#pragma unroll
    for (int o = 4; o < 64; o <<= 1) q += __shfl_xor(q, o, 64);
    if (lane < 4) red[wave][lane] = q;
    __syncthreads();
    const float var = (red[0][tx] + red[1][tx] + red[2][tx] + red[3][tx]) / (float)C;
    const float inv = 1.0f / sqrtf(var + 1e-5f);
    if (ok) {
        float *yp = y + (long long)b * y_bs + t;
#pragma unroll
        for (int i = 0; i < NV; i++) {
            const int c = ty + i * 64;
            if (c < C) yp[(long long)c * y_cs] = (v[i] - mean) * inv * gv[i] + bv[i];
        }
    }
}

static __global__ __launch_bounds__(256) void layernorm_tile_kernel(const float *x, float *y, const float *g, const float *bta,
                                                             int C, int T, int x_cs, long long x_bs, int y_cs, long long y_bs)
{
    extern __shared__ __attribute__((aligned(16))) float tile[];
    __shared__ float red[8][32], s_mean[32], s_inv[32];
    const int t0 = blockIdx.x * 32, b = blockIdx.y, tid = threadIdx.x, tx = tid & 31, part = tid >> 5;
    const float *xb = x + (long long)b * x_bs + t0;
    const bool ok = t0 + tx < T;
    for (int c0 = part; c0 < C; c0 += 8 * 4) {
        float v[4];
#pragma unroll
        for (int u = 0; u < 4; u++) { const int c = c0 + 8 * u; v[u] = (ok && c < C) ? xb[(long long)c * x_cs + tx] : 0.f; }
#pragma unroll
        for (int u = 0; u < 4; u++) { const int c = c0 + 8 * u; if (c < C) tile[c * 33 + tx] = v[u]; }
    }
    __syncthreads();
    float s = 0.f;
    for (int c = part; c < C; c += 8) s += tile[c * 33 + tx];
    red[part][tx] = s;
    __syncthreads();
    if (part == 0) { float m = 0.f; for (int q = 0; q < 8; q++) m += red[q][tx]; s_mean[tx] = m / (float)C; }
    __syncthreads();
    const float mean = s_mean[tx];
    float qv = 0.f;
    for (int c = part; c < C; c += 8) { const float d = tile[c * 33 + tx] - mean; qv += d * d; }
    red[part][tx] = qv;
    __syncthreads();
    if (part == 0) { float m = 0.f; for (int q = 0; q < 8; q++) m += red[q][tx]; s_inv[tx] = 1.0f / sqrtf(m / (float)C + 1e-5f); }
    __syncthreads();
    if (!ok) return;
    const float inv = s_inv[tx];
    float *yb = y + (long long)b * y_bs + t0;
    for (int c = part; c < C; c += 8) yb[(long long)c * y_cs + tx] = (tile[c * 33 + tx] - mean) * inv * g[c] + bta[c];
}

template <int NR>
__global__ __launch_bounds__(256) void layernorm_strip_kernel(const float *x, float *y, const float *g, const float *bta,
                                                              int C, int T, int x_cs, long long x_bs, int y_cs, long long y_bs)
{
    __shared__ float red[64][17];
    __shared__ float s_stat[2][16];
    const int t0 = blockIdx.y * 16, b = blockIdx.x, tid = threadIdx.x, quad = tid & 3, rg = tid >> 2;
    const float *xb = x + (long long)b * x_bs + t0 + quad * 4;
    f32x4 v[NR];
#pragma unroll
    for (int r = 0; r < NR; r++) {
        const int c = rg + r * 64;
        v[r] = c < C ? *reinterpret_cast<const f32x4 *>(xb + (long long)c * x_cs) : (f32x4){0.f, 0.f, 0.f, 0.f};
    }
    f32x4 sm = {0.f, 0.f, 0.f, 0.f};
#pragma unroll
    for (int r = 0; r < NR; r++) sm += v[r];
#pragma unroll
    for (int j = 0; j < 4; j++) red[rg][quad * 4 + j] = sm[j];
    __syncthreads();
    if (tid < 16) { float m = 0.f; for (int q = 0; q < 64; q++) m += red[q][tid]; s_stat[0][tid] = m / (float)C; }
    __syncthreads();
    f32x4 mean;
#pragma unroll
    for (int j = 0; j < 4; j++) mean[j] = s_stat[0][quad * 4 + j];
    f32x4 qv = {0.f, 0.f, 0.f, 0.f};
#pragma unroll
    for (int r = 0; r < NR; r++) { if (rg + r * 64 < C) { const f32x4 d = v[r] - mean; qv += d * d; } }
#pragma unroll
    for (int j = 0; j < 4; j++) red[rg][quad * 4 + j] = qv[j];
    __syncthreads();
    if (tid < 16) { float m = 0.f; for (int q = 0; q < 64; q++) m += red[q][tid]; s_stat[1][tid] = 1.0f / sqrtf(m / (float)C + 1e-5f); }
    __syncthreads();
    f32x4 inv;
#pragma unroll
    for (int j = 0; j < 4; j++) inv[j] = s_stat[1][quad * 4 + j];
    float *yb = y + (long long)b * y_bs + t0 + quad * 4;
    const int tq = t0 + quad * 4;
    if (tq >= T) return;
#pragma unroll
    for (int r = 0; r < NR; r++) {
        const int c = rg + r * 64;
        if (c >= C) break;
        const float gg = g[c], bb = bta[c];
        f32x4 o;
// ... 1853 lines not shown
```

obs_rvc_amd/csrc/model_synth.hip:

```cpp
#include "engine_int.h"

namespace rvc {

void add_nsf_source(Plan &pl, int B, const float *pitchf, const T1 &src, int R, int upp, float sr, float lin_w, float lin_b, const StreamState *st, const CallParams *cp,
                    int f0_num, int f0_den)
{
    if (R > 512) throw ShapeError("return_length too long for the NSF source kernel");
    if (R < 1 || upp < 1 || src.T != R * upp || src.C != 1 || f0_den < 1) throw ShapeError("NSF source: inconsistent shapes");
    SrcP sp{}; sp.pitchf = pitchf; sp.src = src.p; sp.src_bs = src.bs; sp.T = R; sp.upp = upp; sp.sr = sr;
    sp.lin_w = lin_w; sp.lin_b = lin_b; sp.st = st; sp.cp = cp;
    sp.f0_num = f0_num; sp.f0_den = f0_den;
    pl.ops.push_back([=](hipStream_t s) { hipLaunchKernelGGL(nsf_source_kernel, dim3(B), dim3(1024), 0, s, sp); });
}

T1 build_nsf_source(rvc_engine *e, Plan &pl, int B, float *d_pitchf)
{
    ModelSY &m = *e->sy;
    Arena &A = pl.arena;
    const int R = (int)pl.R, R2 = pl.dec_frames();
    const int upp = m.upp();
    const size_t N = (size_t)R * upp;
    if (R > 512) throw ShapeError("return_length too long for the NSF source kernel");
    int max_sf = 1; { int sf = 1; for (int i = m.n_ups - 1; i >= 1; i--) { sf *= m.up_rate[i]; max_sf = std::max(max_sf, sf); } }
    T1 src = make_t1(A, B, 1, (int)N, max_sf + 2);
    add_nsf_source(pl, B, d_pitchf, src, R, upp, (float)m.sr, m.src_w, m.src_b, e->d_state, e->d_cp, R2, R);
    add_tap(pl, "sy.src", src);
    if (!pl.fstage) return src;
    T1 srci = src;
    if (R2 != R) {
        srci = make_t1(A, B, 1, R2 * upp, max_sf + 2);
        const int Nin = (int)N, Nout = R2 * upp; dim3 grid((Nout + 255) / 256, B);
        pl.ops.push_back([=](hipStream_t s) { hipLaunchKernelGGL(time_lerp_kernel, grid, dim3(256), 0, s, src.p, src.ld, src.bs, srci.p, srci.ld, srci.bs, 1, Nin, Nout); });
    }
    add_tap(pl, "sy.srci", srci);
    return srci;
}

std::vector<T1> build_noise_convs(rvc_engine *e, Plan &pl, int B, const T1 &src)
{
    ModelSY &m = *e->sy;
    std::vector<T1> nz;
    int c = m.up_init, Tc = pl.dec_frames();
    for (int i = 0; i < m.n_ups; i++) {
        const int co = c / 2, Tn = Tc * m.up_rate[i];
        T1 t = make_t1(pl.arena, B, co, Tn, 0);
        int sf = 1; for (int q = i + 1; q < m.n_ups; q++) sf *= m.up_rate[q];
        if (i + 1 < m.n_ups) add_conv1d(pl, m.ncs[i], src, t, sf, sf / 2, 1); else add_conv1d(pl, m.ncs[i], src, t, 1, 0, 1);
        nz.push_back(t);
        c = co; Tc = Tn;
    }
    return nz;
}

void build_synth(rvc_engine *e, Plan &pl, int B, const T1 &phone, const T1 &src, float *d_pitchf, int *d_pitch, int src_join_sid,
                        const std::vector<T1> *nz)
{
    ModelSY &m = *e->sy;
    Arena &A = pl.arena;
    const int R = (int)pl.R, H = m.hidden, I = m.inter, F = m.filter, half = I / 2;
    const int HALO = 4;
    if (m.enc_k / 2 > HALO || m.wn_k / 2 > HALO) throw ShapeError("synth kernel sizes exceed the halo");
    T1 z = make_t1(A, B, I, R, HALO), zf = make_t1(A, B, I, R, HALO);
    {
        T1 x = make_t1(A, B, H, R, HALO);
        add_conv1d(pl, m.phone, phone, x, 1, 0, 1);
        {
            dim3 grid((H * R + 255) / 256, B); float *emb = m.pitch_emb; float sq = sqrtf((float)H);
            pl.ops.push_back([=](hipStream_t s) { hipLaunchKernelGGL(embed_pitch_kernel, grid, dim3(256), 0, s, x.p, x.ld, x.bs, emb, d_pitch, H, R, sq); });
        }
        add_tap(pl, "sy.emb", x);
        T1 qkv = make_t1(A, B, 3 * H, R, 0), att = make_t1(A, B, H, R, 0), ff = make_t1(A, B, F, R, HALO);
        const bool fuse_ln = B <= LN_FOLD_MAX_STREAMS && m.has_folded && !pl.plain_plan && !test_opt("RVC_NO_LN_FUSE");
        bool raw = false; const float *raw_g = nullptr, *raw_b = nullptr; float *raw_st = nullptr;
        for (int l = 0; l < m.enc_layers; l++) {
            ModelSY::Layer &Ly = m.layers[l];
            if (raw) { raw_st = A.floats((size_t)2 * R + 16); ConvOpts o; o.ln_wsum = Ly.qkv_wsum; o.ln_stats_out = raw_st; o.ln_rows = H; add_conv1d(pl, Ly.qkv_f, x, qkv, 1, 0, 1, o); }
            else add_conv1d(pl, Ly.qkv, x, qkv, 1, 0, 1);
            add_relpos_attention(pl, qkv, att, m.heads, Ly.rel_k, Ly.rel_v, m.window);
            {
                ConvOpts o; o.res = x.p; o.res_cs = x.ld; o.res_bs = x.bs;
                if (raw) { o.ln_stats_in = raw_st; o.ln_g = raw_g; o.ln_b = raw_b; }
                add_conv1d(pl, Ly.o, att, x, 1, 0, 1, o);
            }
            add_layernorm(pl, x, Ly.ln1_g, Ly.ln1_b);
            { ConvOpts o; o.act = ACT_RELU; add_conv1d(pl, Ly.ff1, x, ff, 1, m.enc_k / 2, 1, o); }
            { ConvOpts o; o.res = x.p; o.res_cs = x.ld; o.res_bs = x.bs; add_conv1d(pl, Ly.ff2, ff, x, 1, m.enc_k / 2, 1, o); }
            if (fuse_ln) { raw = true; raw_g = Ly.ln2_g; raw_b = Ly.ln2_b; }
            else add_layernorm(pl, x, Ly.ln2_g, Ly.ln2_b);
        }
        add_tap(pl, raw ? "sy.enc.raw" : "sy.enc", x);
        static const int wn_max_b = tune_env("RVC_WN_COMPOSE_MAX") ? atoi(tune_env("RVC_WN_COMPOSE_MAX")) : 8;
        const bool wn_composed = B <= wn_max_b && H % 16 == 0 && I == H && !pl.plain_plan && !test_opt("RVC_NO_WN_COMPOSE");
        T1 U[2];
        const int u_z = 16 + H + H * m.wn_layers;
        if (wn_composed) {
            m.compose_flows();
            std::vector<float> ones(R, 1.0f);
            for (int k = 0; k < 2; k++) {
                U[k] = make_t1(A, B, u_z + I, R, HALO);
                for (int bb = 0; bb < B; bb++) HIPCHK(hipMemcpy(U[k].p + (long long)bb * U[k].bs, ones.data(), (size_t)R * sizeof(float), hipMemcpyHostToDevice));
            }
            z = U[0].rows(u_z, I);
        }
        T1 stats = make_t1(A, B, 2 * I, R, 0);
        if (raw) { ConvOpts o; o.ln_wsum = m.proj_wsum; o.ln_rows = H; add_conv1d(pl, m.proj_f, x, stats, 1, 0, 1, o); }
        else add_conv1d(pl, m.proj, x, stats, 1, 0, 1);
        add_tap(pl, "sy.stats", stats);
        {
            dim3 grid(((I * R + 3) / 4 + 255) / 256, B); StreamState *st = e->d_state; CallParams *cp = e->d_cp;
            pl.ops.push_back([=](hipStream_t s) { hipLaunchKernelGGL(prior_sample_kernel, grid, dim3(256), 0, s, stats.p, stats.ld, stats.bs, z.p, z.ld, z.bs, I, R, st, cp); });
        }
        add_tap(pl, "sy.zp", z);
        T1 hs = make_t1(A, B, 2 * H, R, HALO), acts = make_t1(A, B, H, R, 0);
        T1 hh = hs.rows(0, H), skip = hs.rows(H, H);
        for (int fi = m.flow_n - 1; fi >= 0; fi--) {
            ModelSY::Flow &Fw = m.flows[fi];
            const T1 x0 = Fw.flipped ? z.rows(half, half) : z.rows(0, half), x1 = Fw.flipped ? z.rows(0, half) : z.rows(half, half);
            if (wn_composed) {
                const int k = m.flow_n - 1 - fi;
                const T1 &Uc = U[k & 1], &Un = U[(k + 1) & 1];
                if (k == 0) add_conv1d(pl, Fw.pre1, Uc.rows(u_z, I), Uc.rows(16, H), 1, 0, 1);
                for (int j = 0; j < m.wn_layers; j++) { ConvOpts o; o.glu = true; add_conv1d(pl, Fw.inc[j], Uc.rows(0, 16 + H * (j + 1)), Uc.rows(16 + H * (j + 1), H), 1, (m.wn_k - 1) / 2, 1, o); }
                if (fi > 0) add_conv1d_two(pl, Fw.posth, Fw.postc, Fw.pair_bias, Uc.rows(16 + H, H * m.wn_layers + I), Un.rows(16, H), Un.rows(u_z, I));
                else add_conv1d(pl, Fw.postc, Uc.rows(16 + H, H * m.wn_layers + I), Un.rows(u_z, I), 1, 0, 1);
                if (fi == 0) z = Un.rows(u_z, I);
                if (pl.with_taps) { char nm[32]; snprintf(nm, sizeof nm, "sy.flow%d", fi); add_tap(pl, nm, Un.rows(u_z, I)); } else add_stamp(pl, "sy.flow");
                continue;
            }
            add_conv1d(pl, Fw.pre, x0, hs, 1, 0, 1);
            for (int j = 0; j < m.wn_layers; j++) {
                { ConvOpts o; o.glu = true; add_conv1d(pl, Fw.in[j], hh, acts, 1, (m.wn_k - 1) / 2, 1, o); }
                ConvOpts o; o.accumulate = true;
                if (j < m.wn_layers - 1) add_conv1d(pl, Fw.rs[j], acts, hs, 1, 0, 1, o);
                else add_conv1d(pl, Fw.rs[j], acts, skip, 1, 0, 1, o);
            }
            { ConvOpts o; o.scale = -1.f; o.accumulate = true; add_conv1d(pl, Fw.post, skip, x1, 1, 0, 1, o); }
            if (pl.with_taps) { char nm[32]; snprintf(nm, sizeof nm, "sy.flow%d", fi); add_tap(pl, nm, z); } else add_stamp(pl, "sy.flow");
        }
        if (m.flow_n & 1) {
            T1 zi = z, zo = zf; dim3 grid((I * R + 255) / 256, B);
            pl.ops.push_back([=](hipStream_t s) { hipLaunchKernelGGL(flip_channels_kernel, grid, dim3(256), 0, s, zi.p, zi.ld, zi.bs, zo.p, zo.ld, zo.bs, I, R); });
            std::swap(z, zf);
        }
    }
    add_tap(pl, "sy.z", z);
    const int upp = m.upp();
    const int R2 = pl.dec_frames();
    if (pl.fstage) {
        if (R2 != R) {
            T1 zi = make_t1(A, B, I, R2, HALO); dim3 grid((I * R2 + 255) / 256, B); T1 zs = z;
            pl.ops.push_back([=](hipStream_t s) { hipLaunchKernelGGL(time_lerp_kernel, grid, dim3(256), 0, s, zs.p, zs.ld, zs.bs, zi.p, zi.ld, zi.bs, I, R, R2); });
            z = zi;
        }
        add_tap(pl, "sy.zi", z);
    }
    int max_pad = 3;
    for (int j = 0; j < m.n_rb; j++) for (int q = 0; q < m.n_rbd; q++) max_pad = std::max(max_pad, (m.rb_k[j] * m.rb_d[q] - m.rb_d[q]) / 2);
    const int DH = (max_pad + 3) / 4 * 4;
    int c = m.up_init, Tc = R2;
    if (src_join_sid > 0) pl.ops.join(src_join_sid);
    T1 xd = make_t1(A, B, c, Tc, DH);
    add_conv1d(pl, m.dec_pre, z, xd, 1, 3, 1);
    add_tap(pl, "sy.pre", xd);
    for (int i = 0; i < m.n_ups; i++) {
        const int co = c / 2, K = m.up_kernel[i], S = m.up_rate[i], Tn = Tc * S;
        if ((K - S) % 2 != 0) throw ShapeError("upsample kernel/stride parity not supported");
        T1 u = make_t1(A, B, co, Tn, DH);
        if (nz) {
            const T1 &r = (*nz)[i];
            ConvOpts o; o.pre_act = ACT_LRELU; o.pre_slope = 0.1f; o.res = r.p; o.res_cs = r.ld; o.res_bs = r.bs;
            add_convT1d(pl, m.ups[i], xd, u, (K - S) / 2, o);
        } else {
        { ConvOpts o; o.pre_act = ACT_LRELU; o.pre_slope = 0.1f; add_convT1d(pl, m.ups[i], xd, u, (K - S) / 2, o); }
        int sf = 1; for (int q = i + 1; q < m.n_ups; q++) sf *= m.up_rate[q];
        { ConvOpts o; o.accumulate = true; if (i + 1 < m.n_ups) add_conv1d(pl, m.ncs[i], src, u, sf, sf / 2, 1, o); else add_conv1d(pl, m.ncs[i], src, u, 1, 0, 1, o); }
        }
        if (pl.with_taps) { char nm[32]; snprintf(nm, sizeof nm, "sy.up%d", i); add_tap(pl, nm, u); } else add_stamp(pl, "sy.up");
        T1 xs = make_t1(A, B, co, Tn, DH);
        std::vector<T1> finals;
        const bool fused = m.n_rb > 1 && m.n_rb <= 3 && B < 16 && !tune_env("RVC_SERIAL_RESBLOCKS");
        if (fused) {
            const int nr = m.n_rb;
            T1 ra = make_t1(A, B, nr * co, Tn, DH), rb = make_t1(A, B, nr * co, Tn, DH), tt = make_t1(A, B, nr * co, Tn, DH), fin = make_t1(A, B, nr * co, Tn, 0);
            T1 cur = u; bool grouped = false;
            for (int q = 0; q < m.n_rbd; q++) {
                const int d = m.rb_d[q];
                std::vector<const ConvW *> c1, c2; std::vector<int> p1, d1, p2, d2;
                for (int j = 0; j < nr; j++) {
                    c1.push_back(&m.rbs[i][j][q].first); c2.push_back(&m.rbs[i][j][q].second);
                    p1.push_back((m.rb_k[j] * d - d) / 2); d1.push_back(d); p2.push_back((m.rb_k[j] - 1) / 2); d2.push_back(1);
                }
// ... 69 lines not shown
```

obs_rvc_amd/csrc/plan.hip:

```cpp
#include "engine_int.h"
#include <chrono>

namespace rvc {

struct TestHook { const char *name; bool planner; };
static const TestHook kTestHooks[] = {
    {"RVC_FORCE_CFG", true}, {"RVC_CONV_TILE", true}, {"RVC_CONV_TILE_KS", true}, {"RVC_NO_LN_FUSE", false}, {"RVC_NO_CONV0_MULTI", false},
    {"RVC_KNN_NO_GEMM", false}, {"RVC_KNN_EXHAUSTIVE", false}, {"RVC_STAMPS", false}, {"RVC_SERIAL_BRANCHES", false}, {"RVC_NO_WN_COMPOSE", false},
    {"RVC_KNN_LOSE_TICKET", false}, {"RVC_FORCE_G2W", true}, {"RVC_F0_XCDS", false}, {"RVC_CONV32S", true}, {"RVC_CONV32S_TILE", true},
    {"RVC_G32L", true}, {"RVC_G32L_TALL", true}, {"RVC_G32L_TAB", true}, {"RVC_CONV32S_BUF", true}, {"RVC_FORCE_CHOICE", true},
    {"RVC_G32L_PANEL", true}, {"RVC_MEAN3", false}, {"RVC_RM_FUSE", false}, {"RVC_G2W_LN", false}, {"RVC_RELPOS_MFMA_MAX", false},
    {"RVC_ATTN_KERNEL", false}, {"RVC_RELPOS_KERNEL", false}, {"RVC_LN_KERNEL", false}, {"RVC_GRU_KERNEL", false}, {"RVC_CONV0_KERNEL", false}
};
std::atomic<unsigned> g_opt_gen{0};
static std::mutex g_opt_mu;
static std::map<std::string, std::string> g_opts;
static bool is_test_hook(const char *name)
{
    for (const TestHook &h : kTestHooks) if (!strcmp(h.name, name)) return true;
    return false;
}
static const char *opt_lookup(const char *name)
{
    static thread_local std::string buf;
    std::lock_guard<std::mutex> lk(g_opt_mu);
    auto it = g_opts.find(name);
    if (it == g_opts.end()) return nullptr;
    buf = it->second;
    return buf.c_str();
}
#ifdef RVC_TUNING
const char *test_opt(const char *name) { const char *v = opt_lookup(name); return v ? v : getenv(name); }
const char *tune_env(const char *name) { const char *v = opt_lookup(name); return v ? v : getenv(name); }
#else
const char *test_opt(const char *name) { return opt_lookup(name); }
#endif
int test_opt_int(const char *name, int dflt) { const char *v = test_opt(name); return v ? atoi(v) : dflt; }

namespace {
struct WSlab { char *base; size_t size, used; long live; int dev, cls; };
std::mutex g_wslab_mu;
std::vector<WSlab> g_wslabs;
const size_t kWSlabBytes = (size_t)256 << 20, kPlanSlabBytes = (size_t)64 << 20;
void *wmalloc_cls(size_t bytes, int cls)
{
    bytes = (std::max<size_t>(bytes, 16) + 255) / 256 * 256;
    std::lock_guard<std::mutex> lk(g_wslab_mu);
    int dev = 0; HIPCHK(hipGetDevice(&dev));
    const size_t slab = cls ? kPlanSlabBytes : kWSlabBytes;
    if (bytes <= slab / 4) {
        for (size_t i = g_wslabs.size(); i-- > 0; ) {
            WSlab &b = g_wslabs[i];
            if (b.dev == dev && b.cls == cls && b.size == slab && b.used + bytes <= b.size) {
                void *r = b.base + b.used; b.used += bytes; b.live++;
                return r;
            }
        }
    }
    const size_t sz = bytes <= slab / 4 ? slab : bytes;
    void *c;
    HIPCHK(hipMalloc(&c, sz));
    g_wslabs.push_back(WSlab{(char *)c, sz, bytes, 1, dev, cls});
    return c;
}
}
void *wmalloc(size_t bytes) { return wmalloc_cls(bytes, 0); }
void *wmalloc_plan(size_t bytes) { return wmalloc_cls(bytes, 1); }
void wfree(void *p)
{
    if (!p) return;
    std::lock_guard<std::mutex> lk(g_wslab_mu);
    for (size_t i = 0; i < g_wslabs.size(); i++) {
        WSlab &b = g_wslabs[i];
        if ((char *)p >= b.base && (char *)p < b.base + b.size) {
            if (--b.live == 0) { (void)hipFree(b.base); g_wslabs.erase(g_wslabs.begin() + i); }
            return;
        }
    }
    (void)hipFree(p);
}
void wslab_info(int dev, int *count, size_t *bytes)
{
    std::lock_guard<std::mutex> lk(g_wslab_mu);
    *count = 0; *bytes = 0;
    for (const WSlab &b : g_wslabs) if (b.dev == dev) { (*count)++; *bytes += b.size; }
}

float *upload_f(const std::vector<float> &v, int cls)
{
    float *d = (float *)(cls ? wmalloc_plan(std::max<size_t>(v.size(), 4) * sizeof(float)) : wmalloc(std::max<size_t>(v.size(), 4) * sizeof(float)));
    if (!v.empty()) HIPCHK(hipMemcpy(d, v.data(), v.size() * sizeof(float), hipMemcpyHostToDevice));
    return d;
}
float *upload_f(const float *p, size_t n) { return upload_f(std::vector<float>(p, p + n)); }

// ... 94 lines not shown
    float *dst = (float *)wmalloc(n * sizeof(float));
    HIPCHK(hipMemsetAsync(dst + (size_t)mt * nchunks * 256, 0, (size_t)16 * 256 * sizeof(float), nullptr));
    hipLaunchKernelGGL(c32s_repack_kernel, dim3((unsigned)std::min<size_t>((n + 255) / 256, 4096)), dim3(256), 0, nullptr, src_frag, dst, mt, nchunks, KW, cin / 32);
    HIPCHK(hipGetLastError());
    HIPCHK(hipStreamSynchronize(nullptr));
    g_panels[key] = dst;
    return dst;
}
static void c32s_forget(const float *base, size_t elems)
{
    std::lock_guard<std::mutex> lk(g_panel_mu);
    for (auto it = g_panels.begin(); it != g_panels.end();) {
        if (it->first.src >= base && it->first.src < base + elems) { wfree(it->second); it = g_panels.erase(it); }
        else ++it;
    }
}

void free_conv(ConvW &c)
{
    if (c.w) c32s_forget(c.w, (size_t)c.nphase * (size_t)phase_stride(c));
    if (c.owns) {
        if (c.w) wfree(c.w);
        if (c.bias) wfree(c.bias);
    }
    c.w = c.bias = nullptr;
}
void merge_convs(const std::vector<ConvW *> &cs)
{
    size_t tw = 0, tb = 0;
    for (ConvW *c : cs) { if (!c->owns || !c->bias) throw std::runtime_error("merge_convs: unexpected conv"); tw += (size_t)c->nphase * phase_stride(*c); tb += (size_t)c->Cout; }
    float *W, *Bv;
    W = (float *)wmalloc(tw * sizeof(float)); Bv = (float *)wmalloc(std::max<size_t>(tb, 4) * sizeof(float));
    size_t ow = 0, ob = 0;
    for (size_t i = 0; i < cs.size(); i++) {
        ConvW *c = cs[i];
        const size_t nw = (size_t)c->nphase * phase_stride(*c);
        HIPCHK(hipMemcpy(W + ow, c->w, nw * sizeof(float), hipMemcpyDeviceToDevice));
        HIPCHK(hipMemcpy(Bv + ob, c->bias, (size_t)c->Cout * sizeof(float), hipMemcpyDeviceToDevice));
        wfree(c->w); wfree(c->bias);
        c->w = W + ow; c->bias = Bv + ob; c->owns = i == 0;
        ow += nw; ob += c->Cout;
    }
}


unsigned long long *g_kprobe = nullptr;
int g_last_waves = 0, g_last_wgs = 0;
thread_local char g_last_kernel[32] = "";
static void note_kernel(const char *d) { size_t i = 0; for (; i < sizeof(g_last_kernel) - 1 && d[i] && d[i] != ' '; i++) g_last_kernel[i] = d[i]; g_last_kernel[i] = 0; }

template <class Launch> void queue_gemm_launch(Plan &pl, const char *desc, double flops, int wgs, int waves, bool final_out, const IgemmP &p, Launch launch)
{
    pl.descs.push_back(desc); note_kernel(desc);
    g_last_wgs = wgs; g_last_waves = waves;
    pl.igemm_flops += flops; pl.n_igemm++;
    if (final_out) pl.final_out_honoured = true;
    Plan *plp = &pl;
    const int desc_id = (int)pl.descs.size() - 1;
    pl.ops.push_back([=](hipStream_t s) {
        const ProfEvent *pe = plp->prof_slot(flops, 0, desc_id);
        hipEvent_t ea = pe ? pe->a : nullptr, eb = pe ? pe->b : nullptr;
        if (final_out && plp->cur_out) { IgemmP q = p; q.y = plp->cur_out; q.y_bs = plp->cur_out_bs; launch(q, ea, eb, s); }
        else launch(p, ea, eb, s);
    });
}

int g_ncu = 256;

struct Choice {
    int kind = 0;
    int a = 0, b = 0;
    bool operator==(const Choice &o) const { return kind == o.kind && a == o.a && b == o.b; }
};

struct GemmCall {
    Plan &pl;
    const std::vector<int> &koff;
    bool final_out;
    const Choice &ch;
    int streams;
    double ksum = 0;
    bool phase_epi = false;
    bool ln_fold = false;
    Choice built;
};

static void set_phases(Plan &pl, IgemmP &p, const std::vector<PhaseD> &ph) { p.ph = pl.arena.upload(ph); p.nphase = (int)ph.size(); p.ph0 = ph[0]; }

static bool decode_taps(PhaseD &q, const std::vector<int> &koff, const IgemmP &p, int cblk)
{
    const int K = q.nchunks * 16;
    int cin = 1;
    for (int k = 0; k < K; k++) cin = std::max(cin, (int)std::floor((double)koff[q.koff_off + k] / p.x_ld + 0.5) + 1);
    if (cin % cblk != 0 || K % cin != 0) return false;
    const int KW = K / cin;
    if (KW > 255) return false;
    const int dmin = koff[q.koff_off];
    const int dil = KW > 1 ? koff[q.koff_off + 1] - koff[q.koff_off] : 1;
    if (dil < 1 || dil > 255 || dmin > 0 || dmin < p.x_lo) return false;
    for (int k = 0; k < K; k++) if (koff[q.koff_off + k] != (k / KW) * p.x_ld + dmin + (k % KW) * dil) return false;
    q.t_tab = KW | (dil << 8); q.t_cin = cin; q.t_dmin = dmin;
    return true;
}

static bool queue_conv_tile(GemmCall &c, IgemmP p, int B, const std::vector<PhaseD> &phv)
{
    const int mode = c.ch.kind ? 0 : test_opt_int("RVC_CONV_TILE", 1);
    if (!mode || p.fold_n || p.x_ld <= 0 || p.x_hs || p.x_ws != 1 || p.y_hm || p.lin_cs4 || p.glu || p.ln_wsum || p.ln_stats_in || p.ln_stats_out || p.part) return false;
    if (B > 4) return false;
    if (p.M > 128 && mode < 2) return false;
    const int kshares = test_opt_int("RVC_CONV_TILE_KS", 2);
    const int tc0 = p.M > 64 ? 0 : (p.M > 32 ? 1 : 2);
    const int BM = kTileBM[tc0], BN = kTileBN[tc0];
    const int ntm = (p.M + BM - 1) / BM, ntn = (p.N + BN - 1) / BN;
    if (ntm > 255 || ntn > 32767 || phv.size() > 255) return false;
    const long long nitems = (long long)ntm * ntn * (long long)phv.size() * B;
    if (mode < 2 && nitems < 3 * g_ncu / 2) return false;
    std::vector<PhaseD> phs(phv);
    std::vector<float> wnew;
    size_t lds_max = 0;
    const int mt = (p.M + 15) / 16;
    for (PhaseD &q : phs) {
        if (!decode_taps(q, c.koff, p, 16)) return false;
        const int KW = q.t_tab & 0xff, dil = q.t_tab >> 8, cin = q.t_cin;
        const int rl = BN + (KW - 1) * dil, rt = rl | 1, cs = cin + 8;
        q.t_rs = rt;
        if (q.nchunks < 2 || cin / 16 < kshares) return false;
        lds_max = std::max(lds_max, (std::max<size_t>(((size_t)cin * rt + 63) / 64 * 64, (size_t)kTileWF[tc0] * 256) + (size_t)rl * cs) * 4);
        std::vector<float> wold((size_t)mt * q.nchunks * 256);
        HIPCHK(hipMemcpy(wold.data(), p.w + q.w_off, wold.size() * 4, hipMemcpyDeviceToHost));
        const size_t base = wnew.size();
        wnew.resize(base + wold.size());
        const int G = cin / 16;
        for (int t = 0; t < mt; t++)
            for (int tap = 0; tap < KW; tap++)
                for (int g = 0; g < G; g++)
                    for (int l = 0; l < 64; l++)
                        for (int j = 0; j < 4; j++) {
                            const int k = (g * 16 + (l >> 4) * 4 + j) * KW + tap;
                            wnew[base + (((size_t)t * q.nchunks + tap * G + g) * 64 + l) * 4 + j] =
                                wold[(((size_t)t * q.nchunks + k / 16) * 64 + (((k % 16) / 4) << 4 | (l & 15))) * 4 + (k % 4)];
                        }
        q.w_off = (long long)base;
    }
    if (lds_max > 100 * 1024) return false;
    Plan &pl = c.pl;
    wnew.resize(wnew.size() + (size_t)16 * 2 * 256, 0.f);
    p.w = pl.arena.upload(wnew);
    struct It { int w, code, b; };
    std::vector<It> items;
    for (int bb = 0; bb < B; bb++)
        for (size_t f = 0; f < phs.size(); f++)
            for (int tm = 0; tm < ntm; tm++)
                for (int tn = 0; tn < ntn; tn++) items.push_back({phs[f].nchunks + 12, (int)f | (tm << 8) | (tn << 16), bb});
    std::stable_sort(items.begin(), items.end(), [](const It &a, const It &b) { return a.w > b.w; });
    const int nb = g_ncu;
    std::vector<std::vector<int>> bins(nb);
    {
        std::vector<std::pair<long long, int>> heap;
        for (int j = 0; j < nb; j++) heap.push_back({0, j});
        auto cmp = [](const std::pair<long long, int> &a, const std::pair<long long, int> &b) { return a > b; };
        std::make_heap(heap.begin(), heap.end(), cmp);
        for (size_t i = 0; i < items.size(); i++) {
            std::pop_heap(heap.begin(), heap.end(), cmp);
            auto &top = heap.back();
            bins[top.second].push_back((int)i); top.first += items[i].w;
// ... 217 lines not shown
    const int wgs = (int)(grid.x * grid.y);
    const bool g32t = (lc == 3 || lc == 7 || lc == 8) && g32t_on &&
                      !(lc == 3 && pre);
    const bool g32l = ((lc == 3 || lc == 7 || lc == 8) && g32l_on && !(lc == 3 && p.m_fast == 2)) || g32t;
    const int g32l_mode = g32t ? (pre ? 2 : 1) : 0;
    const size_t lds_l = (size_t)2 * bn * 20 * 4;
    if (g32l && !g32t && p.fold_n && B == 1 && (lc == 7 || lc == 8) && p.ntm >= 8 && p.ntn >= 64 && test_opt_int("RVC_G32L_PANEL", 1) != 0) {
        const size_t per_tile = (size_t)bm * (size_t)c.ksum * sizeof(float);
        const int mp = (int)std::max<size_t>(1, ((size_t)5 << 19) / per_tile);
        if ((size_t)p.M * (size_t)c.ksum * sizeof(float) > ((size_t)5 << 19) && mp < p.ntm) {
            p.m_fast = 3; p.pad2_ = mp;
            const int nx_max = (p.ntn + 7) / 8;
            grid = dim3((unsigned)(8 * nx_max * p.ntm), 1u);
        }
    }
    char d[160];
    snprintf(d, sizeof d, "%s M=%d N=%d K=%d B=%d nph=%d tile=%dx%d grid=%ux%u", g32t ? "g32t" : g32l ? "g32l" : g32k ? "g32" : "lds", p.M, p.N, p.K, B, p.nphase, bm, bn, grid.x, grid.y);
    queue_gemm_launch(c.pl, d, 2.0 * p.M * (double)p.N * c.ksum * B, wgs, 4, c.final_out, p,
                      [=](const IgemmP &q, hipEvent_t ea, hipEvent_t eb, hipStream_t s) {
                          if (g32l) launch_igemm32l(lc, g32l_mode, q, grid, lds_l, s, ea, eb);
                          else launch_igemm_tiled(lc, pre, q, grid, lds, s, ea, eb);
                      });
    c.built = Choice{3, lc, 0};
    return true;
}

static void queue_reg(GemmCall &c, IgemmP p, int B, const std::vector<PhaseD> &phv)
{
    const int nchunks = p.K / 16;
    const bool pre = p.pre_act != ACT_NONE;
    auto fits = [&](int cf, int ks) {
        return (ks == 1 || (nchunks / ks >= 4 && ks * kMF[cf] * kNF[cf] <= 32)) && (size_t)nchunks * 64 + (ks > 1 ? (size_t)ks * kMF[cf] * kNF[cf] * 1024 : 0) <= 60 * 1024;
    };
    auto tiles = [&](int cf) {
        long long tm = (p.M + 16 * kMF[cf] - 1) / (16 * kMF[cf]), tn = (p.N + 16 * kNF[cf] - 1) / (16 * kNF[cf]);
        return tm * tn * B * p.nphase;
    };
    const int order_big[3] = {4, 3, 0}, order_small[3] = {2, 1, 0};
    const bool pad32 = p.M > 16 && (((p.M + 31) / 32 * 32 - p.M) * 4 >= p.M);
    const int *order = (p.M > 16 && !pad32) ? order_big : order_small;
    int cfg = 0, wg_ks = 1;
    long long best_waves = -1;
    bool found = false;
    bool uneven = false;
    for (const PhaseD &q : phv) uneven = uneven || q.nchunks != phv[0].nchunks;
    long long want_waves = (uneven && p.M >= 64) ? 2048 : 1024;
    if (const char *f = tune_env("RVC_WANT_WAVES")) { if (p.fold_n) want_waves = atoll(f); }
    for (int oi = 0; oi < 3 && !found; oi++) {
        const int cf = order[oi];
        for (int ks = 1; ks <= 16; ks = ks == 1 ? 4 : ks * 2) {
            if (!fits(cf, ks)) break;
            const long long w = tiles(cf) * ks;
            if (w > best_waves) { best_waves = w; cfg = cf; wg_ks = ks; }
            if (p.fold_n && oi == 0 && !tune_env("RVC_NO_BALANCE")) {
                const long long wgs = ks > 1 ? tiles(cf) : (tiles(cf) + 3) / 4, rounds = (wgs + g_ncu - 1) / g_ncu;
                if (rounds < 4 && wgs * 5 < rounds * g_ncu * 4) continue;
            }
            if (w >= want_waves) { cfg = cf; wg_ks = ks; found = true; break; }
        }
    }
    if (cfg == 0 && wg_ks == 4 && B == 1 && !p.fold_n && p.lin_cs4 && p.nphase == 1 && p.M >= 256 && p.N > 64 && p.N <= 128 && nchunks >= 32 && !p.ln_wsum && !tune_env("RVC_NO_LIN_16x32")) { cfg = 1; wg_ks = 8; }
    if (const char *f = tune_env("RVC_TUNE")) {
        for (const char *q = f; q && *q; ) {
            int tm = 0, tk = 0, tc = 0, tks = 1;
            if (sscanf(q, "%d,%d:%d,%d", &tm, &tk, &tc, &tks) == 4 && tm == p.M && tk == p.K) { cfg = tc; wg_ks = tks; }
            q = strchr(q, ';'); if (q) q++;
        }
    }
    if (const char *f = test_opt("RVC_FORCE_CFG")) {
        int fc = 0, fk = 1; if (sscanf(f, "%d,%d", &fc, &fk) >= 1) { cfg = fc; wg_ks = fk; }
    }
    if (c.ch.kind == 4 && !(p.ln_wsum || p.ln_stats_in)) {
        const int fc = c.ch.a, fk = c.ch.b;
        if (fc >= 0 && fc <= 4 && (fk == 1 || fk == 4 || fk == 8 || fk == 16) && fits(fc, fk)) { cfg = fc; wg_ks = fk; }
    }
    if (p.ln_wsum || p.ln_stats_in) {
        if (B != 1 || p.nphase != 1) throw std::logic_error("folded LayerNorm outside its supported launch shape");
        if (wg_ks == 1) {
            wg_ks = 4;
            while (cfg > 0 && (nchunks / wg_ks < 4 || wg_ks * kMF[cfg] * kNF[cfg] > 32)) cfg = cfg == 4 ? 3 : (cfg == 3 ? 1 : 0);
        }
        if (p.ln_wsum && (p.lin_cs4 == 0 || pre || nchunks / wg_ks < 1)) throw std::logic_error("LayerNorm consumer must be a table-free 1x1 layer");
    }
    int ksplit = 1;
    if ((size_t)nchunks * 64 > 60 * 1024 && (p.glu || c.phase_epi)) throw ShapeError("fused conv too long for the in-workgroup K split");
    if ((size_t)nchunks * 64 > 60 * 1024) {
        ksplit = (int)(((size_t)nchunks * 64 + 60 * 1024 - 1) / (60 * 1024));
        cfg = 0; wg_ks = 1;
    }
    int cps = (nchunks + ksplit - 1) / ksplit;
    ksplit = (nchunks + cps - 1) / cps;
    p.ksplit = ksplit; p.chunks_per_split = cps;
    p.ntm = (p.M + 16 * kMF[cfg] - 1) / (16 * kMF[cfg]);
    p.ntn = (p.N + 16 * kNF[cfg] - 1) / (16 * kNF[cfg]);
    if (ksplit > 1) p.part = c.pl.arena.floats((size_t)B * p.nphase * ksplit * p.M * p.N);
    bool weight_heavy = (p.N <= 512 && (long long)p.M * p.K >= 64 * 1024 && p.ntm >= 8) || (p.fold_n && p.ntm >= 2);
    if (const char *f = tune_env("RVC_FORCE_MFAST")) weight_heavy = atoi(f) != 0;
    p.m_fast = weight_heavy ? (p.ntm + 7) / 8 * 8 : 0;
    const int ntiles = weight_heavy ? p.m_fast * p.ntn : p.ntm * p.ntn;
    dim3 grid(wg_ks > 1 ? ntiles : (ntiles + 3) / 4, B * p.nphase * ksplit);
    dim3 egrid((unsigned)(((long long)p.M * p.N + 255) / 256), B * p.nphase);
    const bool lean = ksplit == 1 && !tune_env("RVC_OLD_IGEMM");
    const bool lin = lean && p.lin_cs4 != 0 && p.nphase == 1 && !pre && !tune_env("RVC_NO_LIN");
    size_t lds2 = 0;
    if (lean) {
        const int fast_n = weight_heavy ? p.ntm : p.ntn, slow_n = weight_heavy ? p.ntn : p.ntm;
        unsigned gx = (unsigned)(wg_ks > 1 ? fast_n : (fast_n + 3) / 4);
        if (weight_heavy && ((wg_ks > 1 && gx >= 8) || gx >= 16)) gx = (gx + 7) / 8 * 8;
        grid = dim3(gx, (unsigned)slow_n, (unsigned)(B * p.nphase));
        if (grid.y > 65535 || grid.z > 65535) throw ShapeError("implicit GEMM grid too large");
        p.nbatch = B;
        lds2 = (lin ? 0 : (size_t)nchunks * 64) + (wg_ks > 1 ? (size_t)wg_ks * kMF[cfg] * kNF[cfg] * 1024 : 0) + (p.ln_wsum ? (size_t)wg_ks * kNF[cfg] * 16 * 2 * 4 : 0);
        if (p.ln_wsum && !lin) throw std::logic_error("LayerNorm consumer did not get the table-free kernel");
    }
    char d[200];
    snprintf(d, sizeof d, "reg M=%d N=%d K=%d B=%d nph=%d tile=%dx%d ks=%d mfast=%d grid=%ux%ux%u pre=%d lin=%d ksum=%.0f", p.M, p.N, p.K, B, p.nphase, 16 * kMF[cfg], 16 * kNF[cfg], wg_ks, p.m_fast, grid.x, grid.y, grid.z, (int)pre, (int)lin, c.ksum);
    queue_gemm_launch(c.pl, d, 2.0 * p.M * (double)p.N * c.ksum * B, (int)(grid.x * grid.y * grid.z), wg_ks > 1 ? wg_ks : 4, c.final_out && lean, p,
                      [=](const IgemmP &q, hipEvent_t ea, hipEvent_t eb, hipStream_t s) {
                          if (lean) { launch_igemm2(cfg, wg_ks, pre, lin, q, grid, lds2, s, ea, eb); return; }
                          if (ea && ksplit > 1) HIPCHK(hipEventRecord(ea, s));
                          launch_igemm_v1(pre, q, grid, s);
                          if (ksplit > 1) hipLaunchKernelGGL(splitk_epilogue_kernel, egrid, dim3(256), 0, s, q);
                          if (eb && ksplit > 1) HIPCHK(hipEventRecord(eb, s));
                      });
    c.built = Choice{4, cfg, wg_ks};
}

static Choice queue_igemm_impl(Plan &pl, IgemmP p, int B, const std::vector<int> &koff, const std::vector<PhaseD> &phases, bool final_out, const Choice &ch)
{
    p.probe = g_kprobe;
    GemmCall c{pl, koff, final_out, ch, B};
    std::vector<PhaseD> ph(phases);
    for (PhaseD &q : ph) {
        if (q.nchunks == 0) q.nchunks = p.K / 16;
        c.ksum += q.nchunks * 16.0;
        c.phase_epi = c.phase_epi || q.act_p1 != 0 || q.y_off != 0;
    }
    c.ln_fold = p.ln_wsum || p.ln_stats_in || c.phase_epi;
    std::vector<PhaseD> lpt(ph);
    std::stable_sort(lpt.begin(), lpt.end(), [](const PhaseD &a, const PhaseD &b) { return a.nchunks > b.nchunks; });
    if (B > 1) {
        if (queue_conv_tile(c, p, B, lpt)) return c.built;
        if (queue_conv32s(c, p, B, lpt)) return c.built;
    }
    if (B == 1 && test_opt_int("RVC_CONV32S", 1) == 2 && queue_conv32s(c, p, B, ph)) return c.built;
    if (B > 1 && !tune_env("RVC_NO_FOLD")) {
        const long long lim = (1LL << 29);
        if ((long long)B * p.x_bs < lim && (long long)B * p.y_bs < lim && (long long)B * (p.res ? p.res_bs : 0) < lim && (long long)B * p.N < (1LL << 30) &&
            (size_t)(p.K / 16) * 64 <= 60 * 1024) {
            p.fold_n = p.N; p.N = B * p.N; B = 1;
        }
    }
    std::vector<int> kb(koff);
    int kmin = 0;
    for (int v : kb) kmin = std::min(kmin, v);
    for (int &v : kb) v = (v - kmin) * 4;
    p.koff_bias = -kmin * 4;
    {
        auto it = pl.koff_tabs.find(kb);
        if (it == pl.koff_tabs.end()) it = pl.koff_tabs.emplace(kb, pl.arena.upload(kb)).first;
        p.koff = it->second;
    }
    if (!tune_env("RVC_NO_LPT")) ph = lpt;
    set_phases(pl, p, ph);
    if (queue_conv_tile(c, p, B, ph) || queue_bf3(c, p, B, ph) || queue_g2w(c, p, B) || queue_tiled(c, p, B)) return c.built;
    queue_reg(c, p, B, ph);
    return c.built;
}

namespace {
struct TuneRec { Choice c; std::string desc; double us; int ncand; };
std::mutex g_tune_mu;
std::map<std::string, TuneRec> g_tune;
std::atomic<long long> g_tune_trials{0};
hipStream_t tune_stream()
{
    static thread_local std::map<int, hipStream_t> st;
    int dev = 0; HIPCHK(hipGetDevice(&dev));
    auto it = st.find(dev);
    if (it != st.end()) return it->second;
    hipStream_t s; HIPCHK(hipStreamCreateWithFlags(&s, hipStreamNonBlocking));
    st[dev] = s;
    return s;
}
bool planner_hook_set()
{
    for (const TestHook &h : kTestHooks) if (h.planner && test_opt(h.name)) return true;
    return false;
}
}

static double tune_trial(const Plan &pl, const IgemmP &p, int B, const std::vector<int> &koff, const std::vector<PhaseD> &phases, const Choice &c, int reps, std::string *desc,
                         Choice *built = nullptr)
{
    static thread_local Plan *scratch = nullptr;
    static thread_local int scratch_dev = -1;
    int dev = 0; HIPCHK(hipGetDevice(&dev));
    if (!scratch || scratch_dev != dev) { delete scratch; scratch = new Plan(); scratch->arena.set_chunk_min((size_t)8 << 20); scratch_dev = dev; }
    Plan &tp = *scratch;
    HIPCHK(hipStreamSynchronize(tune_stream()));
    tp.ops = OpList(); tp.descs.clear(); tp.koff_tabs.clear(); tp.arena.rewind();
    tp.B = pl.B; tp.bf3 = pl.bf3; tp.autotune = false; tp.profile = false; tp.igemm_flops = 0; tp.n_igemm = 0;
    Choice b;
    try { b = queue_igemm_impl(tp, p, B, koff, phases, false, c); }
    catch (...) { return -1.0; }
    if (tp.ops.v.empty() || tp.descs.empty()) return -1.0;
    *desc = tp.descs.back();
    if (built) *built = b;
    hipStream_t st = tune_stream();
    static thread_local hipEvent_t ea = nullptr, eb = nullptr;
    if (!ea) { HIPCHK(hipEventCreate(&ea)); HIPCHK(hipEventCreate(&eb)); }
    Op &op = tp.ops.v.back();
    double best = 1e30;
    for (int r = 0; r <= reps; r++) {
        HIPCHK(hipEventRecord(ea, st));
        op(st);
        HIPCHK(hipEventRecord(eb, st));
        HIPCHK(hipEventSynchronize(eb));
        float ms = 0.f; HIPCHK(hipEventElapsedTime(&ms, ea, eb));
        if (r == 0 && ms < 0.4f) continue;
        best = std::min(best, (double)ms * 1e3);
// ... 46 lines not shown
    const int t32 = p.M <= 32 ? 0 : (p.M <= 64 ? 1 : 2);
    const int lc_m = p.M >= 96 ? 7 : (p.M >= 48 ? 8 : 5);
    const int nchunks = p.K / 16;
    const int g2w_ks = g2w_ksplit(p.M, (long long)B * p.N, nchunks);
    if (b0.kind == 1) {
        add(1, t32 == 2 ? 1 : t32 + 1, 0); if (t32 > 0) add(1, t32 - 1, 0);
        if (t32 == 1) { add(1, 1 | 4, 0); add(1, 1, 0); }
        add(3, lc_m, 0);
    } else if (b0.kind == 2) {
        const int ks = b0.b;
        add(2, 0, ks == 1 ? 2 : ks / 2); if (ks < 8) add(2, 0, ks == 3 ? 4 : ks * 2);
        add(3, p.M >= 96 ? 8 : lc_m, 0); add(4, 3, 4);
    } else if (b0.kind == 3) {
        if (p.M >= 96) { add(3, 7, 0); add(3, 3, 0); add(3, 8, 0); } else if (p.M >= 48) { add(3, 4, 0); add(3, 8, 0); add(3, 5, 0); } else add(3, 5, 0);
        if (one_d && !lin) add(1, t32, 0);
        if (lin && p.M >= 256) add(2, 0, g2w_ks);
        add(4, p.M > 16 ? 3 : 1, nchunks >= 16 ? 4 : 1);
    } else if (b0.kind == 4) {
        if (one_d && !lin) add(1, t32, 0);
        if (lin && p.M >= 256) add(2, 0, g2w_ks);
        if (p.M > 16) add(3, lc_m, 0);
        const int cf = b0.a, ks = b0.b;
        add(4, cf, ks == 1 ? 4 : (ks == 4 ? 8 : 4));
        if (cf == 4 || cf == 3) add(4, cf == 4 ? 3 : 0, ks);
    }
    struct Res { Choice c; std::string d; double us; };
    std::vector<Res> res;
    res.push_back({Choice(), d0, us0});
    for (const Choice &c : cands) {
        std::string d;
        double us = tune_trial(pl, p, B, koff, phases, c, 1, &d);
        if (us < 0) continue;
        bool dup = false;
        for (const Res &r : res) dup = dup || r.d == d;
        if (dup) continue;
        double lead = 1e30; for (const Res &r : res) lead = std::min(lead, r.us);
        if (us < lead * 1.08) us = std::min(us, tune_trial(pl, p, B, koff, phases, c, 2, &d));
        res.push_back({c, d, us});
    }
    size_t bi = 0;
    for (size_t i = 1; i < res.size(); i++) if (res[i].us < res[bi].us) bi = i;
    if (bi != 0 && res[bi].us > res[0].us * 0.985) bi = 0;
    {
        std::lock_guard<std::mutex> lk(g_tune_mu);
        g_tune[key] = TuneRec{res[bi].c, res[bi].d, res[bi].us, (int)res.size()};
    }
    pl.tune_ms += std::chrono::duration<double, std::milli>(std::chrono::steady_clock::now() - t0).count();
    pl.tuned_layers++;
    if (bi != 0) pl.tune_changed++;
    queue_igemm_impl(pl, p, B, koff, phases, final_out, res[bi].c);
}

extern "C" int rvc_debug_autotune_dump(char *buf, size_t cap)
{
    std::lock_guard<std::mutex> lk(g_tune_mu);
    std::string out;
    for (const auto &kv : g_tune) {
        char ln[640];
        snprintf(ln, sizeof ln, "%s -> [%d,%d,%d] %s | %.1f us (%d candidates)\n", kv.first.c_str(), kv.second.c.kind, kv.second.c.a, kv.second.c.b, kv.second.desc.c_str(), kv.second.us, kv.second.ncand);
        out += ln;
    }
    if (buf && out.size() + 1 <= cap) memcpy(buf, out.c_str(), out.size() + 1);
    return (int)g_tune.size();
}
extern "C" void rvc_debug_autotune_reset(void)
{
    std::lock_guard<std::mutex> lk(g_tune_mu);
    g_tune.clear();
}

void fill_epilogue(IgemmP &p, const ConvW &cw, const ConvOpts &o)
{
    p.bias = (o.no_bias || !cw.bias) ? nullptr : cw.bias + o.m_off;
    p.res = o.res; p.res_cs = o.res_cs; p.res_bs = o.res_bs; p.res_rs = o.res_rs;
    p.act = o.act; p.slope = o.slope; p.scale = o.scale; p.accumulate = o.accumulate ? 1 : 0;
    if (o.pre_act != ACT_NONE && o.pre_act != ACT_LRELU) throw std::runtime_error("only LeakyReLU can be fused on the input side");
    p.pre_act = o.pre_act; p.pre_slope = o.pre_act == ACT_LRELU ? o.pre_slope : 1.0f;
    p.part = nullptr;
    p.glu = o.glu ? 1 : 0;
    p.ln_wsum = o.ln_wsum; p.ln_stats_out = o.ln_stats_out; p.ln_stats_in = o.ln_stats_in; p.ln_g = o.ln_g; p.ln_bt = o.ln_b;
    p.ln_eps = 1e-5f; p.ln_inv_rows = o.ln_rows > 0 ? 1.0f / (float)o.ln_rows : 0.f;
    if (o.ln_stats_in && !(o.res && o.ln_g && o.ln_b)) throw std::logic_error("normalised residual without residual / scale / shift");
    if (o.glu && (p.bias == nullptr || o.res || o.accumulate || o.act != ACT_NONE)) throw std::runtime_error("glu epilogue takes bias only");
}

void add_conv1d(Plan &pl, const ConvW &cw, const T1 &x, const T1 &y, int stride, int pad, int dil, ConvOpts o)
{
    if (cw.transposed) throw std::runtime_error("add_conv1d on transposed weights");
    const int cig = cw.Cin / cw.groups, KW = cw.KW;
    const int Tout = (x.T + 2 * pad - dil * (KW - 1) - 1) / stride + 1;
    if (Tout != y.T && !(Tout == y.T + 1)) throw ShapeError("conv1d output length mismatch");
    if (x.halo < pad || (y.T - 1) * stride + (KW - 1) * dil - pad > x.T - 1 + x.halo) throw ShapeError("conv1d halo too small");
    IgemmP p{};
    if (o.m_off % 16 != 0) throw std::runtime_error("output-row sub-range must start at a multiple of 16");
    p.x = x.p; p.w = cw.w + (long long)o.m_off * cw.Kp; p.y = y.p;
    p.M = o.m_cnt >= 0 ? o.m_cnt : cw.M; p.N = y.T; p.K = cw.Kp;
    p.NW = y.T; p.x_hs = 0; p.x_ws = stride; p.y_hm = 0; p.y_ws = 1; p.OW = y.T;
    p.x_bs = x.bs; p.y_bs = y.bs; p.y_cs = y.ld; p.y_rs = 0;
    p.x_ld = x.ld; p.x_lo = -x.halo; p.x_lim = x.T - 1 + x.halo;
    fill_epilogue(p, cw, o);
    p.bf3 = o.bf3 ? 1 : 0;
    if (KW == 1 && cw.groups == 1 && pad == 0 && cw.K == cw.Kp) p.lin_cs4 = x.ld * 4;
    if (cw.groups > 1 && (o.m_off != 0 || o.m_cnt >= 0)) throw std::runtime_error("row sub-range on grouped conv");
    std::vector<int> koff(cw.Kp, 0);
    for (int ci = 0; ci < cig; ci++) for (int k = 0; k < KW; k++) koff[ci * KW + k] = ci * x.ld + k * dil - pad;
    std::vector<PhaseD> ph(cw.groups);
    for (int g = 0; g < cw.groups; g++) {
        ph[g] = PhaseD{};
        ph[g].w_off = (long long)g * phase_stride(cw);
        ph[g].x_off = g * cig * x.ld;
        ph[g].y_c0 = g * cw.M;
        ph[g].y_pos = 0;
        ph[g].bias_off = g * cw.M;
        ph[g].koff_off = 0;
    }
    queue_igemm(pl, p, x.B, koff, ph, o.final_out);
}

void add_conv1d_multi(Plan &pl, const std::vector<const ConvW *> &cws, const T1 &x, bool x_grouped, const T1 &y,
                             const std::vector<int> &pads, const std::vector<int> &dils, ConvOpts o, bool res_grouped)
{
    const int n = (int)cws.size();
    const ConvW &c0 = *cws[0];
    IgemmP p{};
    p.x = x.p; p.w = c0.w; p.y = y.p;
    p.M = c0.M; p.N = y.T; p.K = 0;
    p.NW = y.T; p.x_hs = 0; p.x_ws = 1; p.y_hm = 0; p.y_ws = 1; p.OW = y.T;
    p.x_bs = x.bs; p.y_bs = y.bs; p.y_cs = y.ld; p.y_rs = 0;
    p.x_ld = x.ld; p.x_lo = -x.halo; p.x_lim = x.T - 1 + x.halo;
    fill_epilogue(p, c0, o);
    p.res_nogroup = res_grouped ? 0 : 1;
    std::vector<int> koff;
    std::vector<PhaseD> ph(n);
    for (int j = 0; j < n; j++) {
        const ConvW &cw = *cws[j];
        if (cw.transposed || cw.groups != 1 || cw.Cin != c0.Cin || cw.Cout != c0.Cout || (x_grouped ? x.C != n * cw.Cin : x.C != cw.Cin) || y.C != n * cw.Cout)
            throw std::runtime_error("add_conv1d_multi: incompatible convs");
        const int KW = cw.KW, pad = pads[j], dil = dils[j];
        if (x.T + 2 * pad - dil * (KW - 1) != y.T) throw ShapeError("conv1d_multi output length mismatch");
        if (x.halo < pad || (KW - 1) * dil - pad > x.halo) throw ShapeError("conv1d_multi halo too small");
        ph[j] = PhaseD{};
        ph[j].w_off = cw.w - c0.w;
        ph[j].bias_off = (int)(cw.bias - c0.bias);
        ph[j].x_off = x_grouped ? j * cw.Cin * x.ld : 0;
        ph[j].y_c0 = j * cw.Cout;
        ph[j].koff_off = (int)koff.size();
        ph[j].nchunks = cw.Kp / 16;
        p.K = std::max(p.K, cw.Kp);
        const size_t base = koff.size();
        koff.resize(base + cw.Kp, 0);
        for (int ci = 0; ci < cw.Cin; ci++) for (int k = 0; k < KW; k++) koff[base + ci * KW + k] = ci * x.ld + k * dil - pad;
    }
    queue_igemm(pl, p, x.B, koff, ph);
}

void add_convT1d(Plan &pl, const ConvW &cw, const T1 &x, const T1 &y, int pad, ConvOpts o)
{
    const int S = cw.S, nt = cw.ntaps;
    const int Tout = (x.T - 1) * S - 2 * pad + cw.KW;
    if (Tout != y.T) throw ShapeError("convT1d output length mismatch");
    if (x.halo < nt) throw ShapeError("convT1d halo too small");
    IgemmP p{};
    p.x = x.p; p.w = cw.w; p.y = y.p;
    p.M = cw.M; p.N = x.T + nt - 1; p.K = cw.Kp;
    p.NW = p.N; p.x_hs = 0; p.x_ws = 1; p.y_hm = 0; p.y_ws = S; p.OW = y.T;
    p.x_bs = x.bs; p.y_bs = y.bs; p.y_cs = y.ld; p.y_rs = 0;
// ... 302 lines not shown
```

Baseline: 8055 frames/s.

## Fuse synthesizer glue ops into GEMM epilogues: pitch embed, o-proj+LayerNorm, prior sampling

Adds three fusions in the synthesizer encoder, gated by RVC_GLUE_FUSE (default 6, so two are on by default). The phone projection epilogue now gathers the pitch embedding and applies LeakyReLU. The stats projection now uses GLU-packed rows and samples the prior directly in its epilogue. A dedicated o-proj+residual+LayerNorm kernel (bit 1) is added but left off by default. The goal is fewer small kernel launches and fewer intermediate tensor round trips per chunk. In exchange the epilogue grows more complex, fused shapes are forced to in-workgroup K split, and Philox sampling is recomputed per element.

```diff
diff --git a/include/rvc_mi355x_debug.h b/include/rvc_mi355x_debug.h
--- a/include/rvc_mi355x_debug.h
+++ b/include/rvc_mi355x_debug.h
@@ -12,6 +12,7 @@
 double rvc_debug_conv_check(rvc_engine *e, int M, int Cin, int KW, int dil, int N, int streams, int pre_act);
 double rvc_debug_conv2d_check(rvc_engine *e, int M, int Cin, int H, int W, int streams, int kind, int residual);
 double rvc_debug_ln_fold_check(rvc_engine *e, int M, int K, int N, float offset);
+double rvc_debug_oproj_ln_check(rvc_engine *e, int M, int N, float offset, int ln_in);
 typedef struct rvc_debug_layer_spec {
     int form, streams;
     int cin, cout, kw, stride, pad, dil, groups;
diff --git a/obs_rvc_amd/csrc/engine.hip b/obs_rvc_amd/csrc/engine.hip
--- a/obs_rvc_amd/csrc/engine.hip
+++ b/obs_rvc_amd/csrc/engine.hip
@@ -1213,6 +1213,68 @@
         worst = err;
         free_conv(c1); free_conv(c2);
         wfree(wsum); wfree(dg); wfree(dbeta);
+        return RVC_OK;
+    });
+    return worst;
+}
+
+double rvc_debug_oproj_ln_check(rvc_engine *e, int M, int N, float offset, int ln_in)
+{
+    double worst = -1.0;
+    (void)guarded(e, [&]() {
+        const int K = M;
+        auto rnd = [](size_t i, unsigned salt) { return (float)((((i + 1) * 2654435761u) ^ (salt * 40503u) ^ (i >> 5)) % 2001) / 1000.0f - 1.0f; };
+        std::vector<float> w((size_t)M * K), b(M), g1(M), bt1(M), g2(M), bt2(M), hx((size_t)M * N), ha((size_t)K * N);
+        for (size_t i = 0; i < w.size(); i++) w[i] = 0.5f * rnd(i, 11);
+        for (int m = 0; m < M; m++) { b[m] = 0.1f * rnd(m, 12); g1[m] = 1.0f + 0.3f * rnd(m, 13); bt1[m] = 0.2f * rnd(m, 14); g2[m] = 1.0f + 0.3f * rnd(m, 15); bt2[m] = 0.2f * rnd(m, 16); }
+        for (size_t i = 0; i < hx.size(); i++) hx[i] = 2.0f * rnd(i, 17) + offset;
+        for (size_t i = 0; i < ha.size(); i++) ha[i] = 0.2f * rnd(i, 18);
+        std::vector<double> res((size_t)M * N); std::vector<float> hst((size_t)2 * N);
+        for (int n = 0; n < N; n++) {
+            double s = 0; for (int m = 0; m < M; m++) s += hx[(size_t)m * N + n];
+            const double mu = s / M; double q = 0;
+            for (int m = 0; m < M; m++) { const double d = hx[(size_t)m * N + n] - mu; q += d * d; }
+            const double rs = 1.0 / std::sqrt(q / M + 1e-5);
+            hst[2 * n] = (float)mu; hst[2 * n + 1] = (float)rs;
+            for (int m = 0; m < M; m++) res[(size_t)m * N + n] = ln_in ? (hx[(size_t)m * N + n] - (double)hst[2 * n]) * (double)hst[2 * n + 1] * g2[m] + bt2[m] : (double)hx[(size_t)m * N + n];
+        }
+        ConvW cw = prep_conv(w.data(), b.data(), M, K, 1, 1);
+        float *dg1 = upload_f(g1), *dbt1 = upload_f(bt1), *dg2 = upload_f(g2), *dbt2 = upload_f(bt2), *dst = upload_f(hst);
+        Plan pl; pl.B = 1;
+        T1 x = make_t1(pl.arena, 1, M, N, 4), a = make_t1(pl.arena, 1, K, N, 0);
+        for (int m = 0; m < M; m++) HIPCHK(hipMemcpy(x.p + (long long)m * x.ld, &hx[(size_t)m * N], (size_t)N * 4, hipMemcpyHostToDevice));
+        for (int k = 0; k < K; k++) HIPCHK(hipMemcpy(a.p + (long long)k * a.ld, &ha[(size_t)k * N], (size_t)N * 4, hipMemcpyHostToDevice));
+        const bool taken = add_oproj_ln(pl, cw, a, x, ln_in ? dst : nullptr, ln_in ? dg2 : nullptr, ln_in ? dbt2 : nullptr, dg1, dbt1);
+        if (taken) {
+            HIPCHK(hipDeviceSynchronize());
+            for (auto &op : pl.ops.v) op(e->stream);
+            HIPCHK(hipStreamSynchronize(e->stream));
+            HIPCHK(hipGetLastError());
+            std::vector<double> ref((size_t)M * N); double ss = 0;
+            for (int n = 0; n < N; n++) {
+                std::vector<double> t(M);
+                double s = 0;
+                for (int m = 0; m < M; m++) {
+                    double acc = b[m]; for (int k = 0; k < K; k++) acc += (double)w[(size_t)m * K + k] * ha[(size_t)k * N + n];
+                    t[m] = acc + res[(size_t)m * N + n]; s += t[m];
+                }
+                const double mu = s / M; double q = 0;
+                for (int m = 0; m < M; m++) q += (t[m] - mu) * (t[m] - mu);
+                const double rs = 1.0 / std::sqrt(q / M + 1e-5);
+                for (int m = 0; m < M; m++) { const double v = (t[m] - mu) * rs * g1[m] + bt1[m]; ref[(size_t)m * N + n] = v; ss += v * v; }
+            }
+            const double rms1 = std::sqrt(ss / ((double)M * N)) + 1e-12;
+            double err = 0.0;
+            std::vector<float> row(x.ld);
+            for (int m = 0; m < M; m++) {
+                HIPCHK(hipMemcpy(row.data(), x.p - x.halo + (long long)m * x.ld, (size_t)x.ld * 4, hipMemcpyDeviceToHost));
+                for (int n = 0; n < N; n++) err = std::max(err, std::fabs((double)row[x.halo + n] - ref[(size_t)m * N + n]) / rms1);
+                for (int i = 0; i < x.ld; i++) if ((i < x.halo || i >= x.halo + N) && row[i] != 0.f) err = std::max(err, 1.0);
+            }
+            worst = err;
+        }
+        free_conv(cw);
+        wfree(dg1); wfree(dbt1); wfree(dg2); wfree(dbt2); wfree(dst);
         return RVC_OK;
     });
     return worst;
diff --git a/obs_rvc_amd/csrc/engine_int.h b/obs_rvc_amd/csrc/engine_int.h
--- a/obs_rvc_amd/csrc/engine_int.h
+++ b/obs_rvc_amd/csrc/engine_int.h
@@ -165,6 +165,8 @@
     bool final_out = false;
     const float *ln_wsum = nullptr; float *ln_stats_out = nullptr; int ln_rows = 0;
     const float *ln_stats_in = nullptr, *ln_g = nullptr, *ln_b = nullptr;
+    const int *res_idx = nullptr; float post_slope = 1.f;
+    const StreamState *prior_st = nullptr; const CallParams *prior_cp = nullptr;
 };
 
 struct ProfEvent { hipEvent_t a, b; double flops; double bytes; int desc = -1; };
@@ -256,6 +258,7 @@
 void add_conv2d(Plan &pl, const ConvW &cw, const T2 &x, const T2 &y, ConvOpts o = ConvOpts());
 void add_convT2d(Plan &pl, const ConvW &cw, const T2 &x, const T2 &y, ConvOpts o = ConvOpts());
 void add_layernorm(Plan &pl, const T1 &x, const float *g, const float *b);
+bool add_oproj_ln(Plan &pl, const ConvW &cw, const T1 &att, const T1 &x, const float *stats_in, const float *g_in, const float *b_in, const float *g, const float *bt);
 void add_attention(Plan &pl, const T1 &qkv, const T1 &out, int heads);
 void add_relpos_attention(Plan &pl, const T1 &qkv, const T1 &out, int heads, const float *rel_k, const float *rel_v, int window);
 void add_gru(Plan &pl, const T1 &gi, const T1 &out, int H, const float *whh, const float *whhT, const float *bhh, int *status, int status_stride);
@@ -495,6 +498,7 @@
         ConvW qkv, o, ff1, ff2, qkv_f; float *qkv_wsum = nullptr; float *rel_k, *rel_v, *ln1_g, *ln1_b, *ln2_g, *ln2_b;
     };
     ConvW proj_f; float *proj_wsum = nullptr; bool has_folded = false;
+    ConvW proj_p, proj_fp; float *proj_wsum_p = nullptr; bool has_prior_pack = false;
     std::vector<Layer> layers;
     struct Flow {
         ConvW pre, post; std::vector<ConvW> in, rs; bool flipped = false;
@@ -548,6 +552,14 @@
         proj = prep_conv(b.w("sy.enc.proj.w"), b.w("sy.enc.proj.b"), 2 * inter, H, 1, 1);
         if (has_folded)
             proj_f = ModelCV::fold_ln(b.w("sy.enc.proj.w"), b.w("sy.enc.proj.b"), 2 * inter, H, b.w(fmt("sy.enc.l%d.ln2.g", enc_layers - 1)), b.w(fmt("sy.enc.l%d.ln2.b", enc_layers - 1)), &proj_wsum);
+        if (inter % 8 == 0) {
+            std::vector<float> wp, bp;
+            glu_pack_rows(b.w("sy.enc.proj.w"), b.w("sy.enc.proj.b"), inter, (size_t)H, wp, bp);
+            proj_p = prep_conv(wp.data(), bp.data(), 2 * inter, H, 1, 1);
+            if (has_folded)
+                proj_fp = ModelCV::fold_ln(wp.data(), bp.data(), 2 * inter, H, b.w(fmt("sy.enc.l%d.ln2.g", enc_layers - 1)), b.w(fmt("sy.enc.l%d.ln2.b", enc_layers - 1)), &proj_wsum_p);
+            has_prior_pack = true;
+        }
         const int half = inter / 2;
         for (int i = 0; i < flow_n; i++) {
             Flow F;
@@ -749,6 +761,7 @@
         free_conv(phone); free_conv(proj); free_conv(dec_pre); free_conv(dec_post);
         for (auto &L : layers) { free_conv(L.qkv); free_conv(L.o); free_conv(L.ff1); free_conv(L.ff2); free_conv(L.qkv_f); if (L.qkv_wsum) wfree(L.qkv_wsum); }
         free_conv(proj_f); if (proj_wsum) wfree(proj_wsum);
+        free_conv(proj_p); free_conv(proj_fp); if (proj_wsum_p) wfree(proj_wsum_p);
         for (auto &F : flows) { free_conv(F.pre); free_conv(F.post); for (auto &c : F.in) free_conv(c); for (auto &c : F.rs) free_conv(c); if (composed) { free_conv(F.pre1); free_conv(F.postc); free_conv(F.posth); for (auto &c : F.inc) free_conv(c); } }
         for (auto &c : ups) free_conv(c);
         for (auto &c : ncs) free_conv(c);
diff --git a/obs_rvc_amd/csrc/igemm.hip.h b/obs_rvc_amd/csrc/igemm.hip.h
--- a/obs_rvc_amd/csrc/igemm.hip.h
+++ b/obs_rvc_amd/csrc/igemm.hip.h
@@ -1,6 +1,7 @@
 #pragma once
 #include <hip/hip_runtime.h>
 #include <stdint.h>
+#include "state.hip.h"
 
 namespace rvc {
 
@@ -88,6 +89,9 @@
     float ln_eps, ln_inv_rows;
     const int *items, *ttab;
     int x_ld, x_lo, x_lim, pad2_;
+    const int *res_idx;
+    int post_lrelu; float post_slope;
+    const StreamState *prior_st; const CallParams *prior_cp;
 };
 
 __device__ __forceinline__ void epilogue_store(const IgemmP &p, const PhaseD &ph, int b, int m, int n, float acc)
@@ -116,6 +120,17 @@
     const float ta = a1 + p.bias[ph.bias_off + m1], sa = a2 + p.bias[ph.bias_off + m1 + 2];
     const int ch = (m1 >> 4) * 8 + ((m1 & 15) >> 2) * 2 + (m1 & 1) + ph.y_c0;
     p.y[(long long)b * p.y_bs + (long long)ch * p.y_cs + n] = tanhf(ta) * (1.0f / (1.0f + expf(-sa)));
+}
+
+__device__ __forceinline__ void prior_store(const IgemmP &p, const PhaseD &ph, int b, int m1, int n, float mm, float lg)
+{
+    if (m1 >= p.M || n >= p.N) return;
+    const int ch = (m1 >> 4) * 8 + ((m1 & 15) >> 2) * 2 + (m1 & 1) + ph.y_c0;
+    const int idx = ch * p.N + n, j = idx & 3;
+    float n4[4];
+    philox_normal4(p.prior_cp->seed, p.prior_st[b].stream_id, p.prior_st[b].chunk, 0u, (uint32_t)(idx >> 2), n4);
+    const float eps = j == 0 ? n4[0] : (j == 1 ? n4[1] : (j == 2 ? n4[2] : n4[3]));
+    p.y[(long long)b * p.y_bs + (long long)ch * p.y_cs + n] = mm + expf(lg) * eps * 0.66666f;
 }
 
 struct EpiPre { float bias, res, yold; };
@@ -440,7 +455,8 @@
     if (p.bias) e.bias = p.bias[ph.bias_off + m];
     if (resb) {
         const int rrow = p.res_nogroup ? m : ch;
-        e.res = resb[bb * (int)p.res_bs + rrow * p.res_cs + oh * p.res_rs + ow];
+        if (p.res_idx) e.res = resb[p.res_idx[n_launch] * p.res_cs + m];
+        else e.res = resb[bb * (int)p.res_bs + rrow * p.res_cs + oh * p.res_rs + ow];
         if (p.ln_stats_in)
             e.res = (e.res - p.ln_stats_in[2 * n_launch]) * p.ln_stats_in[2 * n_launch + 1] * p.ln_g[rrow] + p.ln_bt[rrow];
     }
@@ -804,20 +820,6 @@
         RVC_KP(4);
         __syncthreads();
         RVC_KP(5);
-        if (p.glu) {
-#pragma unroll
-            for (int q = 0; q < PE; q++) {
-                const int e = threadIdx.x + q * WAVES * 64;
-                if (e >= TE) break;
-                const int l = e & 63, r = (e >> 6) & 3, f = e >> 8, mf = f / NF, nf = f - mf * NF;
-                if (r >= 2) continue;
-                float v = 0.f, v2 = 0.f;
-#pragma unroll
-                for (int w = 0; w < KS; w++) { v += red[w * TE + e]; v2 += red[w * TE + e + 128]; }
-                glu_store(p, ph, b, tm * 16 * MF + mf * 16 + (l >> 4) * 4 + r, tn * 16 * NF + nf * 16 + (l & 15), v, v2);
-            }
-            return;
-        }
         float ln_mean[LNB ? NF : 1], ln_rstd[LNB ? NF : 1];
         if (LNB) {
 #pragma unroll
@@ -835,6 +837,31 @@
                 if (p.ln_stats_out && tm == 0 && threadIdx.x < 16 && n_ < p.N) { p.ln_stats_out[2 * n_] = mean; p.ln_stats_out[2 * n_ + 1] = rstd; }
             }
         }
+        if (p.glu) {
+#pragma unroll
+            for (int q = 0; q < PE; q++) {
+                const int e = threadIdx.x + q * WAVES * 64;
+                if (e >= TE) break;
+                const int l = e & 63, r = (e >> 6) & 3, f = e >> 8, mf = f / NF, nf = f - mf * NF;
+                if (r >= 2) continue;
+                float v = 0.f, v2 = 0.f;
+#pragma unroll
+                for (int w = 0; w < KS; w++) { v += red[w * TE + e]; v2 += red[w * TE + e + 128]; }
+                const int m1 = tm * 16 * MF + mf * 16 + (l >> 4) * 4 + r, n1 = tn * 16 * NF + nf * 16 + (l & 15);
+                if (p.glu == 2) {
+                    if (m1 < p.M && n1 < p.N) {
+                        if (LNB) {
+                            v = ln_rstd[LNB ? nf : 0] * (v - ln_mean[LNB ? nf : 0] * p.ln_wsum[ph.bias_off + m1]);
+                            v2 = ln_rstd[LNB ? nf : 0] * (v2 - ln_mean[LNB ? nf : 0] * p.ln_wsum[ph.bias_off + m1 + 2]);
+                        }
+                        prior_store(p, ph, b, m1, n1, v + p.bias[ph.bias_off + m1], v2 + p.bias[ph.bias_off + m1 + 2]);
+                    }
+                    continue;
+                }
+                glu_store(p, ph, b, m1, n1, v, v2);
+            }
+            return;
+        }
         float vsum[PE];
 #pragma unroll
         for (int q = 0; q < PE; q++) {
@@ -849,6 +876,15 @@
                 v = ln_rstd[LNB ? nf : 0] * (v - ln_mean[LNB ? nf : 0] * pre_ws[LNB ? q : 0]);
             }
             vsum[q] = v;
+        }
+        if (p.post_lrelu) {
+#pragma unroll
+            for (int q = 0; q < PE; q++) {
+                if (pre_r[q].yo < 0) continue;
+                const float v = epi2_value<ACT_NONE>(vsum[q], pre_r[q].bias, pre_r[q].res, pre_r[q].yold, p.slope, p.scale);
+                yb[pre_r[q].yo] = v > 0.f ? v : v * p.post_slope;
+            }
+            return;
         }
         RVC_ACT_DISPATCH_SEL(act_sel, 
             _Pragma("unroll") for (int q = 0; q < PE; q++) epi2_finish<A_>(p, yb, vsum[q], pre_r[q]);
diff --git a/obs_rvc_amd/csrc/kernels.hip.h b/obs_rvc_amd/csrc/kernels.hip.h
--- a/obs_rvc_amd/csrc/kernels.hip.h
+++ b/obs_rvc_amd/csrc/kernels.hip.h
@@ -199,6 +199,90 @@
             const int c = ty + i * 64;
             if (c < C) yp[(long long)c * y_cs] = (v[i] - mean) * inv * gv[i] + bv[i];
         }
+    }
+}
+
+struct OprojLnP {
+    const float *a, *w, *bias, *stats_in, *g_in, *b_in, *g, *bt;
+    float *x;
+    int a_ld, x_ld, M, N, nchunks;
+    long long a_bs, x_bs;
+    float eps;
+};
+template <int NCH>
+__global__ __launch_bounds__(NCH ? NCH * 64 : 1024) void oproj_ln_kernel(OprojLnP p)
+{
+    __shared__ float red[2][16][16];
+    const int lane = threadIdx.x & 63, wave = threadIdx.x >> 6, nw = blockDim.x >> 6;
+    const int li = lane & 15, kq = lane >> 4, b = blockIdx.y;
+    const int n = blockIdx.x * 16 + li, nc = n < p.N ? n : p.N - 1;
+    const int nch = NCH ? NCH : p.nchunks;
+    const float *ap = p.a + (long long)b * p.a_bs + (long long)(kq * 4) * p.a_ld + nc;
+    const float *wp = p.w + (long long)wave * nch * 256 + lane * 4;
+    float *xp = p.x + (long long)b * p.x_bs + nc;
+    const int m0 = wave * 16 + kq * 4;
+    f32x4 acc0 = {0.f, 0.f, 0.f, 0.f}, acc1 = {0.f, 0.f, 0.f, 0.f};
+    float v[4], gv[4], bv[4];
+    if (NCH) {
+        f32x4 av[NCH ? NCH : 1]; float bq[NCH ? NCH : 1][4];
+#pragma unroll
+        for (int c = 0; c < NCH; c++) {
+            av[c] = *reinterpret_cast<const f32x4 *>(wp + c * 256);
+#pragma unroll
+            for (int j = 0; j < 4; j++) bq[c][j] = ap[(long long)(c * 16 + j) * p.a_ld];
+        }
+#pragma unroll
+        for (int r = 0; r < 4; r++) { v[r] = xp[(long long)(m0 + r) * p.x_ld]; gv[r] = p.g[m0 + r]; bv[r] = p.bt[m0 + r]; }
+        __builtin_amdgcn_sched_barrier(0);
+#pragma unroll
+        for (int c = 0; c < NCH; c++) {
+            acc0 = __builtin_amdgcn_mfma_f32_16x16x4f32(av[c][0], bq[c][0], acc0, 0, 0, 0);
+            acc1 = __builtin_amdgcn_mfma_f32_16x16x4f32(av[c][1], bq[c][1], acc1, 0, 0, 0);
+            acc0 = __builtin_amdgcn_mfma_f32_16x16x4f32(av[c][2], bq[c][2], acc0, 0, 0, 0);
+            acc1 = __builtin_amdgcn_mfma_f32_16x16x4f32(av[c][3], bq[c][3], acc1, 0, 0, 0);
+        }
+    } else {
+#pragma unroll
+        for (int r = 0; r < 4; r++) { v[r] = xp[(long long)(m0 + r) * p.x_ld]; gv[r] = p.g[m0 + r]; bv[r] = p.bt[m0 + r]; }
+        for (int c = 0; c < nch; c++) {
+            const f32x4 av = *reinterpret_cast<const f32x4 *>(wp + c * 256);
+            float bq[4];
+#pragma unroll
+            for (int j = 0; j < 4; j++) bq[j] = ap[(long long)(c * 16 + j) * p.a_ld];
+            acc0 = __builtin_amdgcn_mfma_f32_16x16x4f32(av[0], bq[0], acc0, 0, 0, 0);
+            acc1 = __builtin_amdgcn_mfma_f32_16x16x4f32(av[1], bq[1], acc1, 0, 0, 0);
+            acc0 = __builtin_amdgcn_mfma_f32_16x16x4f32(av[2], bq[2], acc0, 0, 0, 0);
+            acc1 = __builtin_amdgcn_mfma_f32_16x16x4f32(av[3], bq[3], acc1, 0, 0, 0);
+        }
+    }
+    acc0 += acc1;
+    float s = 0.f;
+#pragma unroll
+    for (int r = 0; r < 4; r++) {
+        float res = v[r];
+        if (p.stats_in) res = (res - p.stats_in[2 * nc]) * p.stats_in[2 * nc + 1] * p.g_in[m0 + r] + p.b_in[m0 + r];
+        v[r] = acc0[r] + p.bias[m0 + r];
+        v[r] += res;
+        s += v[r];
+    }
+    s += __shfl_xor(s, 16, 64); s += __shfl_xor(s, 32, 64);
+    if (kq == 0) red[0][wave][li] = s;
+    __syncthreads();
+    float tot = 0.f;
+    for (int w = 0; w < nw; w++) tot += red[0][w][li];
+    const float mean = tot / (float)p.M;
+    float q = 0.f;
+#pragma unroll
+    for (int r = 0; r < 4; r++) { v[r] -= mean; q += v[r] * v[r]; }
+    q += __shfl_xor(q, 16, 64); q += __shfl_xor(q, 32, 64);
+    if (kq == 0) red[1][wave][li] = q;
+    __syncthreads();
+    tot = 0.f;
+    for (int w = 0; w < nw; w++) tot += red[1][w][li];
+    const float inv = 1.0f / sqrtf(tot / (float)p.M + p.eps);
+    if (n < p.N) {
+#pragma unroll
+        for (int r = 0; r < 4; r++) xp[(long long)(m0 + r) * p.x_ld] = v[r] * inv * gv[r] + bv[r];
     }
 }
 
diff --git a/obs_rvc_amd/csrc/model_synth.hip b/obs_rvc_amd/csrc/model_synth.hip
--- a/obs_rvc_amd/csrc/model_synth.hip
+++ b/obs_rvc_amd/csrc/model_synth.hip
@@ -52,6 +52,31 @@
     return nz;
 }
 
+bool add_oproj_ln(Plan &pl, const ConvW &cw, const T1 &att, const T1 &x, const float *stats_in, const float *g_in, const float *b_in, const float *g, const float *bt)
+{
+    if (x.B != 1 || cw.KW != 1 || cw.groups != 1 || cw.transposed || cw.K != cw.Kp || cw.M % 16 != 0 || cw.M > 256 || !cw.bias) return false;
+    if (att.C != cw.K || x.C != cw.M || att.T != x.T || x.T < 1) return false;
+    OprojLnP q{};
+    q.a = att.p; q.a_ld = att.ld; q.a_bs = att.bs; q.w = cw.w; q.bias = cw.bias;
+    q.x = x.p; q.x_ld = x.ld; q.x_bs = x.bs;
+    q.stats_in = stats_in; q.g_in = g_in; q.b_in = b_in; q.g = g; q.bt = bt;
+    q.M = cw.M; q.N = x.T; q.nchunks = cw.Kp / 16; q.eps = 1e-5f;
+    const dim3 grid((unsigned)((x.T + 15) / 16), (unsigned)x.B), block((unsigned)(cw.M / 16 * 64));
+    const double flops = 2.0 * cw.M * (double)x.T * cw.K;
+    pl.igemm_flops += flops; pl.n_igemm++;
+    { char d[176]; snprintf(d, sizeof d, "oln M=%d N=%d K=%d B=1 nph=1 tile=%dx16 grid=%ux%u ln_in=%d", cw.M, x.T, cw.K, cw.M, grid.x, grid.y, stats_in ? 1 : 0); pl.descs.push_back(d); }
+    const int desc_id = (int)pl.descs.size() - 1;
+    const bool k12 = q.nchunks == 12 && cw.M == 192;
+    Plan *plp = &pl;
+    pl.ops.push_back([=](hipStream_t s) {
+        const ProfEvent *pe = plp->prof_slot(flops, 0, desc_id);
+        hipEvent_t ea = pe ? pe->a : nullptr, eb = pe ? pe->b : nullptr;
+        if (k12) { if (ea) hipExtLaunchKernelGGL(oproj_ln_kernel<12>, grid, block, 0, s, ea, eb, 0, q); else hipLaunchKernelGGL(oproj_ln_kernel<12>, grid, block, 0, s, q); }
+        else { if (ea) hipExtLaunchKernelGGL(oproj_ln_kernel<0>, grid, block, 0, s, ea, eb, 0, q); else hipLaunchKernelGGL(oproj_ln_kernel<0>, grid, block, 0, s, q); }
+    });
+    return true;
+}
+
 void build_synth(rvc_engine *e, Plan &pl, int B, const T1 &phone, const T1 &src, float *d_pitchf, int *d_pitch, int src_join_sid,
                         const std::vector<T1> *nz)
 {
@@ -63,8 +88,12 @@
     T1 z = make_t1(A, B, I, R, HALO), zf = make_t1(A, B, I, R, HALO);
     {
         T1 x = make_t1(A, B, H, R, HALO);
-        add_conv1d(pl, m.phone, phone, x, 1, 0, 1);
-        {
+        const int glue = (B == 1 && !pl.plain_plan) ? test_opt_int("RVC_GLUE_FUSE", 6) : 0;
+        if (glue & 2) {
+            ConvOpts o; o.res = m.pitch_emb; o.res_cs = H; o.res_idx = d_pitch; o.scale = sqrtf((float)H); o.post_slope = 0.1f;
+            add_conv1d(pl, m.phone, phone, x, 1, 0, 1, o);
+        } else {
+            add_conv1d(pl, m.phone, phone, x, 1, 0, 1);
             dim3 grid((H * R + 255) / 256, B); float *emb = m.pitch_emb; float sq = sqrtf((float)H);
             pl.ops.push_back([=](hipStream_t s) { hipLaunchKernelGGL(embed_pitch_kernel, grid, dim3(256), 0, s, x.p, x.ld, x.bs, emb, d_pitch, H, R, sq); });
         }
@@ -80,9 +109,11 @@
             {
                 ConvOpts o; o.res = x.p; o.res_cs = x.ld; o.res_bs = x.bs;
                 if (raw) { o.ln_stats_in = raw_st; o.ln_g = raw_g; o.ln_b = raw_b; }
-                add_conv1d(pl, Ly.o, att, x, 1, 0, 1, o);
-            }
-            add_layernorm(pl, x, Ly.ln1_g, Ly.ln1_b);
+                if (!((glue & 1) && add_oproj_ln(pl, Ly.o, att, x, o.ln_stats_in, o.ln_g, o.ln_b, Ly.ln1_g, Ly.ln1_b))) {
+                    add_conv1d(pl, Ly.o, att, x, 1, 0, 1, o);
+                    add_layernorm(pl, x, Ly.ln1_g, Ly.ln1_b);
+                }
+            }
             { ConvOpts o; o.act = ACT_RELU; add_conv1d(pl, Ly.ff1, x, ff, 1, m.enc_k / 2, 1, o); }
             { ConvOpts o; o.res = x.p; o.res_cs = x.ld; o.res_bs = x.bs; add_conv1d(pl, Ly.ff2, ff, x, 1, m.enc_k / 2, 1, o); }
             if (fuse_ln) { raw = true; raw_g = Ly.ln2_g; raw_b = Ly.ln2_b; }
@@ -103,10 +134,17 @@
             z = U[0].rows(u_z, I);
         }
         T1 stats = make_t1(A, B, 2 * I, R, 0);
-        if (raw) { ConvOpts o; o.ln_wsum = m.proj_wsum; o.ln_rows = H; add_conv1d(pl, m.proj_f, x, stats, 1, 0, 1, o); }
-        else add_conv1d(pl, m.proj, x, stats, 1, 0, 1);
+        const bool prior_fused = (glue & 4) && m.has_prior_pack && (!raw || m.proj_wsum_p);
+        if (!prior_fused || pl.with_taps) {
+            if (raw) { ConvOpts o; o.ln_wsum = m.proj_wsum; o.ln_rows = H; add_conv1d(pl, m.proj_f, x, stats, 1, 0, 1, o); }
+            else add_conv1d(pl, m.proj, x, stats, 1, 0, 1);
+        }
         add_tap(pl, "sy.stats", stats);
-        {
+        if (prior_fused) {
+            ConvOpts o; o.glu = true; o.prior_st = e->d_state; o.prior_cp = e->d_cp;
+            if (raw) { o.ln_wsum = m.proj_wsum_p; o.ln_rows = H; add_conv1d(pl, m.proj_fp, x, z, 1, 0, 1, o); }
+            else add_conv1d(pl, m.proj_p, x, z, 1, 0, 1, o);
+        } else {
             dim3 grid(((I * R + 3) / 4 + 255) / 256, B); StreamState *st = e->d_state; CallParams *cp = e->d_cp;
             pl.ops.push_back([=](hipStream_t s) { hipLaunchKernelGGL(prior_sample_kernel, grid, dim3(256), 0, s, stats.p, stats.ld, stats.bs, z.p, z.ld, z.bs, I, R, st, cp); });
         }
diff --git a/obs_rvc_amd/csrc/plan.hip b/obs_rvc_amd/csrc/plan.hip
--- a/obs_rvc_amd/csrc/plan.hip
+++ b/obs_rvc_amd/csrc/plan.hip
@@ -10,7 +10,8 @@
     {"RVC_KNN_LOSE_TICKET", false}, {"RVC_FORCE_G2W", true}, {"RVC_F0_XCDS", false}, {"RVC_CONV32S", true}, {"RVC_CONV32S_TILE", true},
     {"RVC_G32L", true}, {"RVC_G32L_TALL", true}, {"RVC_G32L_TAB", true}, {"RVC_CONV32S_BUF", true}, {"RVC_FORCE_CHOICE", true},
     {"RVC_G32L_PANEL", true}, {"RVC_MEAN3", false}, {"RVC_RM_FUSE", false}, {"RVC_G2W_LN", false}, {"RVC_RELPOS_MFMA_MAX", false},
-    {"RVC_ATTN_KERNEL", false}, {"RVC_RELPOS_KERNEL", false}, {"RVC_LN_KERNEL", false}, {"RVC_GRU_KERNEL", false}, {"RVC_CONV0_KERNEL", false}
+    {"RVC_ATTN_KERNEL", false}, {"RVC_RELPOS_KERNEL", false}, {"RVC_LN_KERNEL", false}, {"RVC_GRU_KERNEL", false}, {"RVC_CONV0_KERNEL", false},
+    {"RVC_GLUE_FUSE", false}
 };
 std::atomic<unsigned> g_opt_gen{0};
 static std::mutex g_opt_mu;
@@ -271,6 +272,7 @@
     double ksum = 0;
     bool phase_epi = false;
     bool ln_fold = false;
+    bool epi_ext = false;
     Choice built;
 };
 
@@ -654,8 +656,9 @@
         }
         if (p.ln_wsum && (p.lin_cs4 == 0 || pre || nchunks / wg_ks < 1)) throw std::logic_error("LayerNorm consumer must be a table-free 1x1 layer");
     }
+    if (c.epi_ext && wg_ks == 1) wg_ks = 4;
     int ksplit = 1;
-    if ((size_t)nchunks * 64 > 60 * 1024 && (p.glu || c.phase_epi)) throw ShapeError("fused conv too long for the in-workgroup K split");
+    if ((size_t)nchunks * 64 > 60 * 1024 && (p.glu || c.phase_epi || c.epi_ext)) throw ShapeError("fused conv too long for the in-workgroup K split");
     if ((size_t)nchunks * 64 > 60 * 1024) {
         ksplit = (int)(((size_t)nchunks * 64 + 60 * 1024 - 1) / (60 * 1024));
         cfg = 0; wg_ks = 1;
@@ -708,7 +711,9 @@
         c.ksum += q.nchunks * 16.0;
         c.phase_epi = c.phase_epi || q.act_p1 != 0 || q.y_off != 0;
     }
-    c.ln_fold = p.ln_wsum || p.ln_stats_in || c.phase_epi;
+    c.epi_ext = p.res_idx || p.post_lrelu || p.glu == 2;
+    if (c.epi_ext && (B != 1 || ph.size() != 1)) throw std::logic_error("folded glue epilogue outside its supported launch shape");
+    c.ln_fold = p.ln_wsum || p.ln_stats_in || c.phase_epi || c.epi_ext;
     std::vector<PhaseD> lpt(ph);
     std::stable_sort(lpt.begin(), lpt.end(), [](const PhaseD &a, const PhaseD &b) { return a.nchunks > b.nchunks; });
     if (B > 1) {
@@ -921,6 +926,13 @@
     p.ln_eps = 1e-5f; p.ln_inv_rows = o.ln_rows > 0 ? 1.0f / (float)o.ln_rows : 0.f;
     if (o.ln_stats_in && !(o.res && o.ln_g && o.ln_b)) throw std::logic_error("normalised residual without residual / scale / shift");
     if (o.glu && (p.bias == nullptr || o.res || o.accumulate || o.act != ACT_NONE)) throw std::runtime_error("glu epilogue takes bias only");
+    p.res_idx = o.res_idx; p.post_lrelu = o.post_slope != 1.f ? 1 : 0; p.post_slope = o.post_slope;
+    if (o.res_idx && (!o.res || o.ln_stats_in)) throw std::logic_error("gathered residual without its table");
+    if (p.post_lrelu && (o.act != ACT_NONE || o.glu)) throw std::logic_error("post-activation behind another activation");
+    if (o.prior_st) {
+        if (!o.glu || !o.prior_cp) throw std::logic_error("prior-sample epilogue takes GLU-packed rows and the call parameters");
+        p.glu = 2; p.prior_st = o.prior_st; p.prior_cp = o.prior_cp;
+    }
 }
 
 void add_conv1d(Plan &pl, const ConvW &cw, const T1 &x, const T1 &y, int stride, int pad, int dil, ConvOpts o)
```

Result: no change. 8077 frames/s, median of 4 (+0.3%).
